# Rudrabha/Wav2Lip

Measured on NVIDIA H100. Metric: 96x96 face-crops/sec (B=128, T=5, mel 80x16), higher is better.
Workload: dtype f16

## Files before the change

wav2lip_b200/csrc/conv_igemm.cuh:

```cuda
#pragma once

#include <cuda.h>
#include <cuda_bf16.h>
#include <cuda_fp16.h>
#include <stdint.h>

#include "wgmma.cuh"

namespace w2l {

constexpr int kTileM = 128;
constexpr int kMaxTaps = 49;
constexpr int kMaxSteps = 3 * kMaxTaps;
constexpr int kSmemExtra = 2048;
constexpr int kSmemMax = 227 * 1024;

enum : int { ACT_NONE = 0, ACT_RELU = 1, ACT_LRELU = 2 };

struct EpiParams {
    int Wout, Hout, N;
    int act;
    int out_f32;
    void* out;
    long long out_sn, out_sy, out_sx;
    const void* res;
    long long res_sn, res_sy, res_sx;
    const float* scale;
    const float* shift;
    const float* head_w;
    const float* head_b;
    int x2;
    int out_lo_off, res_lo_off;
    float* head_out;
    unsigned char* head_out_u8;
    int head_B, head_T;
};

struct alignas(64) ConvParams {
    CUtensorMap tmA;
    CUtensorMap tmB;
    CUtensorMap tmO;
    CUtensorMap tmR;
    int tma_epi;
    unsigned epi_box_bytes;
    int tiles_x, tiles_y, tiles_n, n_tiles;
    int bw, bh, bn;
    int sx, sy;
    int ntaps, kc_per_tap;
    unsigned stage_tx_bytes;
    EpiParams ep;
    int a_lo_off;
    signed char dx[kMaxSteps];
    signed char dy[kMaxSteps];
    unsigned char a_lo[kMaxSteps];
    unsigned char b_slab[kMaxSteps];
};

__device__ __forceinline__ uint32_t smem_u32(const void* p) {
    return static_cast<uint32_t>(__cvta_generic_to_shared(p));
}
__device__ __forceinline__ void mbar_init(uint32_t bar, uint32_t count) {
    asm volatile("mbarrier.init.shared::cta.b64 [%0], %1;" ::"r"(bar), "r"(count) : "memory");
}
__device__ __forceinline__ void mbar_arrive(uint32_t bar) {
    asm volatile("mbarrier.arrive.shared::cta.b64 _, [%0];" ::"r"(bar) : "memory");
}
__device__ __forceinline__ void mbar_arrive_expect_tx(uint32_t bar, uint32_t bytes) {
    asm volatile("mbarrier.arrive.expect_tx.shared::cta.b64 _, [%0], %1;" ::"r"(bar), "r"(bytes) : "memory");
}
__device__ __forceinline__ void mbar_wait(uint32_t bar, uint32_t parity) {
    asm volatile(
        "{\n\t"
        ".reg .pred p;\n\t"
        "W2L_WAIT_%=:\n\t"
        "mbarrier.try_wait.parity.shared::cta.b64 p, [%0], %1;\n\t"
        "@p bra W2L_DONE_%=;\n\t"
        "bra W2L_WAIT_%=;\n\t"
        "W2L_DONE_%=:\n\t"
        "}" ::"r"(bar), "r"(parity)
        : "memory");
}
__device__ __forceinline__ void fence_barrier_init() {
    asm volatile("fence.mbarrier_init.release.cluster;" ::: "memory");
}
__device__ __forceinline__ void tma_prefetch_desc(const void* desc) {
    asm volatile("prefetch.tensormap [%0];" ::"l"(reinterpret_cast<uint64_t>(desc)) : "memory");
}
__device__ __forceinline__ void tma_load_4d(uint32_t dst, const void* desc, uint32_t bar, int c0, int c1, int c2,
                                            int c3) {
    asm volatile(
        "cp.async.bulk.tensor.4d.shared::cluster.global.mbarrier::complete_tx::bytes [%0], [%1, {%3, %4, %5, %6}], [%2];"
        ::"r"(dst), "l"(reinterpret_cast<uint64_t>(desc)), "r"(bar), "r"(c0), "r"(c1), "r"(c2), "r"(c3)
        : "memory");
}
__device__ __forceinline__ void tma_load_3d(uint32_t dst, const void* desc, uint32_t bar, int c0, int c1, int c2) {
    asm volatile(
        "cp.async.bulk.tensor.3d.shared::cluster.global.mbarrier::complete_tx::bytes [%0], [%1, {%3, %4, %5}], [%2];"
        ::"r"(dst), "l"(reinterpret_cast<uint64_t>(desc)), "r"(bar), "r"(c0), "r"(c1), "r"(c2)
        : "memory");
}
__device__ __forceinline__ void pdl_launch_dependents() { asm volatile("griddepcontrol.launch_dependents;" ::: "memory"); }
__device__ __forceinline__ void pdl_wait() { asm volatile("griddepcontrol.wait;" ::: "memory"); }

template <int BK>
__device__ __forceinline__ uint64_t make_kmajor_desc(uint32_t saddr) {
    return wg_desc(saddr, 16, 8 * BK * 2, BK * 2);
}

template <int BN, int BK, bool kBF16>
__device__ __forceinline__ void wg_mma_tile(float (&acc)[2][BN / 2], uint32_t a, uint32_t sbo_a, uint32_t b, bool accumulate) {
#pragma unroll
    for (int k = 0; k < BK / 16; ++k) {
        const uint64_t bd = make_kmajor_desc<BK>(b + 32u * k);
        const uint32_t on = (accumulate || k > 0) ? 1u : 0u;
        wgmma_m64k16<BN, kBF16>(acc[0], wg_desc(a + 32u * k, 16, sbo_a, BK * 2), bd, on, 0);
        wgmma_m64k16<BN, kBF16>(acc[1], wg_desc(a + 8u * sbo_a + 32u * k, 16, sbo_a, BK * 2), bd, on, 0);
    }
}

constexpr int kCmPixels = 256;
template <int BN, int BK, int MT = 1, bool kCM = false>
struct ConvCfg {
    static constexpr int kRowsA = kCM ? kCmPixels : kTileM;
    static constexpr int kATile = kRowsA * BK * 2;
    static constexpr int kABytes = MT * kATile;
    static constexpr int kBBytes = BN * BK * 2;
    static constexpr int kStageBytes = kABytes + kBBytes;
    static constexpr int kEW = BN < 64 ? BN : 64;
    static constexpr int kCW = BN < 32 ? BN : 32;
    static constexpr int kPasses = kCM ? 1 : BN / kEW;
    static constexpr int kBoxBytes = kRowsA * kEW * 2;
    static constexpr int kGrpRaw = (kCM || kPasses * kBoxBytes > xbuf_bytes<kCW>()) ? kPasses * kBoxBytes : xbuf_bytes<kCW>();
    static constexpr int kGrpBytes = (kGrpRaw + 1023) / 1024 * 1024;
    static constexpr int kStagesRaw = (kSmemMax - kSmemExtra - 2 * kGrpBytes) / kStageBytes;
    static constexpr int kStages = kStagesRaw > 8 ? 8 : kStagesRaw;
    static constexpr int kRingBytes = (kStages * kStageBytes + 1023) / 1024 * 1024;
    static constexpr int kSmemBytes = kRingBytes + 2 * kGrpBytes + kSmemExtra;
    static constexpr int kThreads = 384;
    static_assert(BN <= 128, "a warpgroup holds at most 128 fp32 accumulator columns per row");
    static_assert(!kCM || (BN == 128 && BK == 64 && MT == 1), "channel-major form: 128 channels, 128-byte K rows, one tile");
    static_assert(kBoxBytes % 1024 == 0, "staging boxes must keep the 1024-byte swizzle alignment");
    static_assert(kStages >= 2, "need a pipeline");
    static_assert(kSmemBytes <= kSmemMax, "shared-memory carve-up exceeds the per-CTA limit");
};

__device__ int g_f16_overflow = 0;

template <bool kBF16>
__device__ __forceinline__ uint32_t pack2_live(float a, float b, uint32_t live_bits) {
    if constexpr (kBF16) {
        __nv_bfloat162 h = __floats2bfloat162_rn(a, b);
        return *reinterpret_cast<uint32_t*>(&h);
    } else {
        __half2 h = __floats2half2_rn(a, b);
        const uint32_t u = *reinterpret_cast<uint32_t*>(&h);
        if (((u & 0x7FFF7FFFu) + 0x04000400u) & live_bits) g_f16_overflow = 1;
        return u;
    }
}
template <bool kBF16>
__device__ __forceinline__ uint32_t pack2(float a, float b, bool live = true) {
    return pack2_live<kBF16>(a, b, live ? 0x80008000u : 0u);
}
template <bool kBF16>
__device__ __forceinline__ float2 unpack2(uint32_t u) {
    if constexpr (kBF16) {
        return __bfloat1622float2(*reinterpret_cast<__nv_bfloat162*>(&u));
    } else {
        return __half22float2(*reinterpret_cast<__half2*>(&u));
    }
}

template <int BN, bool kBF16, bool kHead>
__device__ __forceinline__ void epilogue_tile(const EpiParams& e, const float (&acc)[2][BN / 2], float* xb, uint32_t bar_id,
                                              bool valid, int n, int y, int x, int nt) {
    constexpr int CH = (BN >= 32) ? 32 : 16;
    const long long o_off = (long long)n * e.out_sn + (long long)y * e.out_sy + (long long)x * e.out_sx;
    const long long r_off = (long long)n * e.res_sn + (long long)y * e.res_sy + (long long)x * e.res_sx;
#pragma unroll
    for (int c0 = 0; c0 < BN; c0 += CH) {
        uint32_t v[CH];
        acc_to_rows<CH>(acc[0], acc[1], c0, xb, bar_id, v);
        if (valid) {
            const int cg = nt * BN + c0;
            float f[CH];
#pragma unroll
            for (int j = 0; j < CH; j += 4) {
                const float4 sc = __ldg(reinterpret_cast<const float4*>(e.scale + cg + j));
                const float4 sh = __ldg(reinterpret_cast<const float4*>(e.shift + cg + j));
                f[j + 0] = fmaf(__uint_as_float(v[j + 0]), sc.x, sh.x);
                f[j + 1] = fmaf(__uint_as_float(v[j + 1]), sc.y, sh.y);
                f[j + 2] = fmaf(__uint_as_float(v[j + 2]), sc.z, sh.z);
                f[j + 3] = fmaf(__uint_as_float(v[j + 3]), sc.w, sh.w);
            }
            if (e.res != nullptr) {
                const uint4* rp = reinterpret_cast<const uint4*>(
                    reinterpret_cast<const uint16_t*>(e.res) + r_off + cg);
#pragma unroll
                for (int j = 0; j < CH / 8; ++j) {
                    const uint4 r = __ldg(rp + j);
                    const float2 a = unpack2<kBF16>(r.x), b = unpack2<kBF16>(r.y);
                    const float2 c = unpack2<kBF16>(r.z), d = unpack2<kBF16>(r.w);
                    f[8 * j + 0] += a.x; f[8 * j + 1] += a.y; f[8 * j + 2] += b.x; f[8 * j + 3] += b.y;
                    f[8 * j + 4] += c.x; f[8 * j + 5] += c.y; f[8 * j + 6] += d.x; f[8 * j + 7] += d.y;
                }
                if (e.x2) {
#pragma unroll
                    for (int j = 0; j < CH / 8; ++j) {
                        const uint4 r = __ldg(rp + (e.res_lo_off >> 3) + j);
                        const float2 a = unpack2<kBF16>(r.x), b = unpack2<kBF16>(r.y);
                        const float2 c = unpack2<kBF16>(r.z), d = unpack2<kBF16>(r.w);
                        f[8 * j + 0] += a.x; f[8 * j + 1] += a.y; f[8 * j + 2] += b.x; f[8 * j + 3] += b.y;
                        f[8 * j + 4] += c.x; f[8 * j + 5] += c.y; f[8 * j + 6] += d.x; f[8 * j + 7] += d.y;
                    }
                }
            }
            if (e.act == ACT_RELU) {
#pragma unroll
                for (int j = 0; j < CH; ++j) f[j] = fmaxf(f[j], 0.0f);
            } else if (e.act == ACT_LRELU) {
#pragma unroll
                for (int j = 0; j < CH; ++j) f[j] = f[j] > 0.0f ? f[j] : 0.01f * f[j];
            }
            if constexpr (kHead) {
                const int hb = n % e.head_B, ht = n / e.head_B;
                const long long plane = (long long)e.Hout * e.Wout;
#pragma unroll
                for (int oc = 0; oc < 3; ++oc) {
                    float s = __ldg(e.head_b + oc);
#pragma unroll
                    for (int j = 0; j < 32; ++j) s = fmaf(f[j], __ldg(e.head_w + oc * 32 + j), s);
                    s = 1.0f / (1.0f + __expf(-s));
                    if (e.head_out_u8 != nullptr)
                        e.head_out_u8[(((long long)n * e.Hout + y) * e.Wout + x) * 3 + oc] = (unsigned char)__fmul_rn(s, 255.0f);
                    else
                        e.head_out[(((long long)hb * 3 + oc) * e.head_T + ht) * plane + (long long)y * e.Wout + x] = s;
                }
            } else if (e.out_f32) {
                float4* op = reinterpret_cast<float4*>(reinterpret_cast<float*>(e.out) + o_off + cg);
#pragma unroll
                for (int j = 0; j < CH / 4; ++j) op[j] = make_float4(f[4 * j], f[4 * j + 1], f[4 * j + 2], f[4 * j + 3]);
            } else {
                uint4* op = reinterpret_cast<uint4*>(reinterpret_cast<uint16_t*>(e.out) + o_off + cg);
#pragma unroll
                for (int j = 0; j < CH / 8; ++j) {
                    uint4 o;
                    o.x = pack2<kBF16>(f[8 * j + 0], f[8 * j + 1]);
                    o.y = pack2<kBF16>(f[8 * j + 2], f[8 * j + 3]);
                    o.z = pack2<kBF16>(f[8 * j + 4], f[8 * j + 5]);
                    o.w = pack2<kBF16>(f[8 * j + 6], f[8 * j + 7]);
                    op[j] = o;
                    if (e.x2) {
                        const float2 h0 = unpack2<kBF16>(o.x), h1 = unpack2<kBF16>(o.y);
                        const float2 h2 = unpack2<kBF16>(o.z), h3 = unpack2<kBF16>(o.w);
                        uint4 l;
                        l.x = pack2<kBF16>(f[8 * j + 0] - h0.x, f[8 * j + 1] - h0.y);
                        l.y = pack2<kBF16>(f[8 * j + 2] - h1.x, f[8 * j + 3] - h1.y);
                        l.z = pack2<kBF16>(f[8 * j + 4] - h2.x, f[8 * j + 5] - h2.y);
                        l.w = pack2<kBF16>(f[8 * j + 6] - h3.x, f[8 * j + 7] - h3.y);
                        op[(e.out_lo_off >> 3) + j] = l;
                    }
                }
            }
        }
    }
}

__device__ __forceinline__ void named_bar_sync(uint32_t id, uint32_t n) { asm volatile("bar.sync %0, %1;" ::"r"(id), "r"(n) : "memory"); }
__device__ __forceinline__ void named_bar_arrive(uint32_t id, uint32_t n) { asm volatile("bar.arrive %0, %1;" ::"r"(id), "r"(n) : "memory"); }

template <bool kBF16, typename AfterRes, typename Live>
__device__ __forceinline__ void chmajor_epilogue(float (&acc)[128], float sc0, float sh0, float sc1, float sh1, int act,
                                                 uint32_t res, int res_pitch, AfterRes&& after_res, Live&& live, uint32_t stg,
                                                 uint32_t bar_id, bool leader, const CUtensorMap* tmO, int c0, int c1, int c2,
                                                 int c3) {
    constexpr uint32_t kRowB = 128;
    const int lane = threadIdx.x & 31, q = (threadIdx.x >> 5) & 3;
    const int lm_row = lane >> 4, lm_px = lane & 7;
    const uint32_t lm_chunk = 16u * (2 * q + ((lane >> 3) & 1));
#pragma unroll
    for (int i = 0; i < 16; ++i) {
#pragma unroll
        for (int h = 0; h < 2; ++h) {
            float* a = acc + 8 * i + 4 * h;
            a[0] = fmaf(a[0], sc0, sh0); a[1] = fmaf(a[1], sc0, sh0);
            a[2] = fmaf(a[2], sc1, sh1); a[3] = fmaf(a[3], sc1, sh1);
        }
        if (res != 0) {
            uint32_t ad = res + static_cast<uint32_t>((2 * i + lm_row) * res_pitch + lm_px) * kRowB + lm_chunk;
            ad ^= ((ad >> 7) & 7u) << 4;
            uint32_t rv[4];
            asm volatile("ldmatrix.sync.aligned.m8n8.x4.trans.shared.b16 {%0,%1,%2,%3}, [%4];"
                         : "=r"(rv[0]), "=r"(rv[1]), "=r"(rv[2]), "=r"(rv[3]) : "r"(ad));
#pragma unroll
            for (int m = 0; m < 4; ++m) {
                const float2 v = unpack2<kBF16>(rv[m]);
                acc[8 * i + 2 * m] += v.x;
                acc[8 * i + 2 * m + 1] += v.y;
            }
        }
    }
    after_res();
    if (act == ACT_RELU) {
#pragma unroll
        for (int j = 0; j < 128; ++j) acc[j] = fmaxf(acc[j], 0.0f);
    } else if (act == ACT_LRELU) {
#pragma unroll
        for (int j = 0; j < 128; ++j) acc[j] = acc[j] > 0.0f ? acc[j] : 0.01f * acc[j];
    }
    if (leader) asm volatile("cp.async.bulk.wait_group.read 0;" ::: "memory");
    named_bar_sync(bar_id, 128);
#pragma unroll
    for (int i = 0; i < 16; ++i) {
        uint32_t ad = stg + static_cast<uint32_t>((2 * i + lm_row) * 8 + lm_px) * kRowB + lm_chunk;
        ad ^= ((ad >> 7) & 7u) << 4;
        const uint32_t l0 = live(2 * i), l1 = live(2 * i + 1);
        const uint32_t o0 = pack2_live<kBF16>(acc[8 * i + 0], acc[8 * i + 1], l0);
        const uint32_t o1 = pack2_live<kBF16>(acc[8 * i + 2], acc[8 * i + 3], l0);
        const uint32_t o2 = pack2_live<kBF16>(acc[8 * i + 4], acc[8 * i + 5], l1);
        const uint32_t o3 = pack2_live<kBF16>(acc[8 * i + 6], acc[8 * i + 7], l1);
        asm volatile("stmatrix.sync.aligned.m8n8.x4.trans.shared.b16 [%0], {%1,%2,%3,%4};"
                     ::"r"(ad), "r"(o0), "r"(o1), "r"(o2), "r"(o3) : "memory");
    }
    asm volatile("fence.proxy.async.shared::cta;" ::: "memory");
    named_bar_sync(bar_id, 128);
    if (leader) {
        asm volatile("cp.async.bulk.tensor.4d.global.shared::cta.bulk_group [%0, {%2, %3, %4, %5}], [%1];"
                     ::"l"(reinterpret_cast<uint64_t>(tmO)), "r"(stg), "r"(c0), "r"(c1), "r"(c2), "r"(c3)
                     : "memory");
        asm volatile("cp.async.bulk.commit_group;" ::: "memory");
    }
}

constexpr int kProducerRegs = 40, kConsumerRegs = 232;
template <int kRegs>
__device__ __forceinline__ void setmaxnreg_dec() { asm volatile("setmaxnreg.dec.sync.aligned.u32 %0;" ::"n"(kRegs)); }
template <int kRegs>
__device__ __forceinline__ void setmaxnreg_inc() { asm volatile("setmaxnreg.inc.sync.aligned.u32 %0;" ::"n"(kRegs)); }

template <int BN, int BK, bool kBF16, bool kHead, int MT = 1, bool kCM = false>
__global__ void __launch_bounds__(ConvCfg<BN, BK, MT, kCM>::kThreads, 1) conv_igemm_kernel(const __grid_constant__ ConvParams p) {
    pdl_launch_dependents();
    using Cfg = ConvCfg<BN, BK, MT, kCM>;
    constexpr int kStages = Cfg::kStages;
    static_assert(!kHead || BN == 32, "fused head expects the 32-channel output block");
    static_assert(MT == 1 || MT == 2, "one or two M tiles per unit");
    static_assert(!kCM || !kHead, "the channel-major form stages its epilogue");

    extern __shared__ uint8_t smem_raw[];
    const uint32_t smem_raw_u32 = smem_u32(smem_raw);
    const uint32_t smem_base = (smem_raw_u32 + 1023u) & ~1023u;
    const uint32_t grp_base = smem_base + Cfg::kRingBytes;
    const uint32_t bar_base = grp_base + 2 * Cfg::kGrpBytes;
    auto full_bar = [&](int s) { return bar_base + 8u * s; };
    auto empty_bar = [&](int s) { return bar_base + 8u * (kStages + s); };
    auto res_bar = [&](int g) { return bar_base + 8u * (2 * kStages + g); };

    const int warp = threadIdx.x >> 5;
    const int lane = threadIdx.x & 31;

    if (warp == 0 && lane == 0) {
        tma_prefetch_desc(&p.tmA);
        tma_prefetch_desc(&p.tmB);
        if (p.tma_epi) {
            tma_prefetch_desc(&p.tmO);
            tma_prefetch_desc(&p.tmR);
        }
    }
    if (warp == 1 && lane == 0) {
        for (int s = 0; s < kStages; ++s) {
            mbar_init(full_bar(s), 1);
            mbar_init(empty_bar(s), kCM ? 8 : 4 * MT);
        }
        for (int g = 0; g < 2; ++g) mbar_init(res_bar(g), 1);
        fence_barrier_init();
    }
    __syncthreads();
    pdl_wait();

    const int m_tiles = p.tiles_x * p.tiles_y * p.tiles_n;
    const int m_units = (m_tiles + MT - 1) / MT;
    const int total_tiles = m_units * p.n_tiles;
    const int k_steps = p.ntaps * p.kc_per_tap;

    if (warp < 4) {
        setmaxnreg_dec<kProducerRegs>();
        if (warp == 0 && lane == 0) {
            int stage = 0;
            uint32_t phase = 0;
            for (int tile = blockIdx.x; tile < total_tiles; tile += gridDim.x) {
                const int nt = tile % p.n_tiles;
                const int mu = tile / p.n_tiles;
                int x_in0[MT], y_in0[MT], n0[MT];
#pragma unroll
                for (int mt = 0; mt < MT; ++mt) {
                    const int m = mu * MT + mt;
                    const int tx = m % p.tiles_x;
                    const int ty = (m / p.tiles_x) % p.tiles_y;
                    const int tn = m / (p.tiles_x * p.tiles_y);
                    x_in0[mt] = tx * p.bw * p.sx;
                    y_in0[mt] = ty * p.bh * p.sy;
                    n0[mt] = tn * p.bn;
                }
                for (int t = 0; t < p.ntaps; ++t) {
                    for (int kc = 0; kc < p.kc_per_tap; ++kc) {
                        mbar_wait(empty_bar(stage), phase ^ 1u);
                        const uint32_t a_dst = smem_base + stage * Cfg::kStageBytes;
                        const uint32_t b_dst = a_dst + Cfg::kABytes;
                        mbar_arrive_expect_tx(full_bar(stage), p.stage_tx_bytes);
#pragma unroll
                        for (int mt = 0; mt < MT; ++mt)
                            tma_load_4d(a_dst + mt * Cfg::kATile, &p.tmA, full_bar(stage), kc * BK + (p.a_lo[t] ? p.a_lo_off : 0),
                                        x_in0[mt] + p.dx[t], y_in0[mt] + p.dy[t], n0[mt]);
                        tma_load_3d(b_dst, &p.tmB, full_bar(stage), kc * BK, nt * BN, p.b_slab[t]);
                        if (++stage == kStages) { stage = 0; phase ^= 1u; }
                    }
                }
            }
        }
    } else if constexpr (kCM) {
        setmaxnreg_inc<kConsumerRegs>();
        const int g = (warp - 4) >> 2;
        const int q = (warp - 4) & 3;
        const uint32_t bar_id = 1 + g;
        const bool leader = (q == 0 && lane == 0);
        const uint32_t stg = grp_base + g * Cfg::kGrpBytes;
        const bool has_res = p.ep.res != nullptr;
        const int rows_valid = p.bw * p.bh * p.bn;
        const int ch = 64 * g + 16 * q + (lane >> 2);
        auto tile_origin = [&](int tile_, int* nt_, int* x0_, int* y0_, int* n0_) {
            *nt_ = tile_ % p.n_tiles;
            const int m_ = tile_ / p.n_tiles;
            *x0_ = (m_ % p.tiles_x) * p.bw;
            *y0_ = ((m_ / p.tiles_x) % p.tiles_y) * p.bh;
            *n0_ = (m_ / (p.tiles_x * p.tiles_y)) * p.bn;
        };
        auto fetch_res = [&](int tile_) {
            int nt_, x0_, y0_, n0_;
            tile_origin(tile_, &nt_, &x0_, &y0_, &n0_);
            mbar_arrive_expect_tx(res_bar(g), p.epi_box_bytes);
            tma_load_4d(stg, &p.tmR, res_bar(g), nt_ * BN + 64 * g, x0_, y0_, n0_);
        };
        if (has_res && leader && static_cast<int>(blockIdx.x) < total_tiles) fetch_res(blockIdx.x);
        float acc[128];
        int stage = 0;
        uint32_t phase = 0, rphase = 0;
        for (int tile = blockIdx.x; tile < total_tiles; tile += gridDim.x) {
            int prev = -1;
            for (int ks = 0; ks < k_steps; ++ks) {
                mbar_wait(full_bar(stage), phase);
                const uint32_t box = smem_base + stage * Cfg::kStageBytes;
                const uint32_t wts = box + Cfg::kABytes + g * (64 * BK * 2);
                wg_fence();
#pragma unroll
                for (int k = 0; k < BK / 16; ++k)
                    wgmma_m64k16<256, kBF16>(acc, make_kmajor_desc<BK>(wts + 32u * k), make_kmajor_desc<BK>(box + 32u * k),
                                             (ks | k) != 0 ? 1u : 0u, 0);
                wg_commit();
                wg_wait<1>();
                if (prev >= 0 && lane == 0) mbar_arrive(empty_bar(prev));
                prev = stage;
                if (++stage == kStages) { stage = 0; phase ^= 1u; }
            }
            wg_wait<0>();
            wg_fence_regs<128>(acc);
            if (lane == 0) mbar_arrive(empty_bar(prev));

            int nt, x0, y0, n0;
            tile_origin(tile, &nt, &x0, &y0, &n0);
            uint64_t live = ~0ull;
            if constexpr (!kBF16) {
                const int xr = p.ep.Wout - x0, yr = p.ep.Hout - y0, nr = p.ep.N - n0;
                if (rows_valid < kCmPixels || xr < p.bw || yr < p.bh || nr < p.bn) {
                    live = 0;
#pragma unroll 1
                    for (int b = 0; b < 64; ++b) {
                        const int px = 8 * (b >> 1) + 2 * (lane & 3) + (b & 1);
                        const int xx = px % p.bw, yy = (px / p.bw) % p.bh, nn = px / (p.bw * p.bh);
                        if (px < rows_valid && xx < xr && yy < yr && nn < nr) live |= 1ull << b;
                    }
                }
            }
            if (has_res) {
                mbar_wait(res_bar(g), rphase);
                rphase ^= 1u;
            }
            const float* const sc = p.ep.scale + nt * BN + ch;
            const float* const sh = p.ep.shift + nt * BN + ch;
            chmajor_epilogue<kBF16>(
                acc, __ldg(sc), __ldg(sh), __ldg(sc + 8), __ldg(sh + 8), p.ep.act, has_res ? stg : 0u, 8, [] {},
                [&](int j) {
                    return (static_cast<uint32_t>(live >> (2 * j)) & 1u) << 15 | (static_cast<uint32_t>(live >> (2 * j + 1)) & 1u) << 31;
                },
                stg, bar_id, leader, &p.tmO, nt * BN + 64 * g, x0, y0, n0);
            if (has_res && leader && tile + static_cast<int>(gridDim.x) < total_tiles) {
                asm volatile("cp.async.bulk.wait_group.read 0;" ::: "memory");
                fetch_res(tile + gridDim.x);
            }
        }
        if (leader) asm volatile("cp.async.bulk.wait_group 0;" ::: "memory");
    } else {
        setmaxnreg_inc<kConsumerRegs>();
        const int g = (warp - 4) >> 2;
        const int q = (warp - 4) & 3;
        const int mt = MT == 2 ? g : 0;
        constexpr int kItStride = MT == 2 ? 1 : 2;
        const int it0 = MT == 2 ? 0 : g;
        const int rows_valid = p.bw * p.bh * p.bn;
        const uint32_t bar_id = 1 + g;
        const uint32_t my_turn = 3 + g, their_turn = 3 + (g ^ 1);
        const uint32_t grp = grp_base + g * Cfg::kGrpBytes;
        float acc[2][BN / 2];
        auto mainloop = [&](int s0, bool hand_off) {
            int stage = s0 % kStages;
            uint32_t phase = static_cast<uint32_t>(s0 / kStages) & 1u;
            int prev = -1;
            for (int ks = 0; ks < k_steps; ++ks) {
                mbar_wait(full_bar(stage), phase);
                const uint32_t a_addr = smem_base + stage * Cfg::kStageBytes + mt * Cfg::kATile;
                wg_fence();
                wg_mma_tile<BN, BK, kBF16>(acc, a_addr, 8 * BK * 2, smem_base + stage * Cfg::kStageBytes + Cfg::kABytes, ks > 0);
                wg_commit();
                wg_wait<1>();
                if (prev >= 0 && lane == 0) mbar_arrive(empty_bar(prev));
                prev = stage;
                if (++stage == kStages) { stage = 0; phase ^= 1u; }
            }
            if (hand_off) named_bar_arrive(their_turn, 256);
            wg_wait<0>();
            wg_fence_regs<BN / 2>(acc[0]);
            wg_fence_regs<BN / 2>(acc[1]);
            if (prev >= 0 && lane == 0) mbar_arrive(empty_bar(prev));
        };
        auto for_each_tile = [&](auto&& epilogue) {
            for (int it = it0;; it += kItStride) {
                const int tile = blockIdx.x + it * static_cast<int>(gridDim.x);
                if (tile >= total_tiles) break;
                if (MT == 1 && it > 0) named_bar_sync(my_turn, 256);
                mainloop(it * k_steps, MT == 1 && tile + static_cast<int>(gridDim.x) < total_tiles);
                epilogue(tile, tile + kItStride * static_cast<int>(gridDim.x) < total_tiles);
            }
        };
        auto tile_origin = [&](int tile_, int* nt_, int* x0_, int* y0_, int* n0_) {
            *nt_ = tile_ % p.n_tiles;
            const int m_ = (tile_ / p.n_tiles) * MT + mt;
            *x0_ = (m_ % p.tiles_x) * p.bw;
            *y0_ = ((m_ / p.tiles_x) % p.tiles_y) * p.bh;
            *n0_ = (m_ / (p.tiles_x * p.tiles_y)) * p.bn;
        };
        if (!kHead && p.tma_epi) {
            constexpr int EW = Cfg::kEW;
            constexpr int kPasses = Cfg::kPasses;
            constexpr uint32_t kRowB = EW * 2;
            constexpr uint32_t kSwz = (kRowB == 128) ? 7u : (kRowB == 64) ? 3u : 1u;
            const bool leader = (q == 0 && lane == 0);
            const bool has_res = p.ep.res != nullptr;
            const EpiParams& e = p.ep;
            auto fetch_res = [&](int tile_) {
                int nt_, x0_, y0_, n0_;
                tile_origin(tile_, &nt_, &x0_, &y0_, &n0_);
                mbar_arrive_expect_tx(res_bar(g), kPasses * p.epi_box_bytes);
#pragma unroll
                for (int ps = 0; ps < kPasses; ++ps)
                    tma_load_4d(grp + ps * Cfg::kBoxBytes, &p.tmR, res_bar(g), nt_ * BN + ps * EW, x0_, y0_, n0_);
            };
            if (has_res && leader) {
                const int first = blockIdx.x + it0 * static_cast<int>(gridDim.x);
                if (first < total_tiles) fetch_res(first);
            }
            uint32_t rphase = 0;
            for_each_tile([&](int tile, bool more) {
                int nt, x0, y0, n0;
                tile_origin(tile, &nt, &x0, &y0, &n0);
                if (has_res) {
                    mbar_wait(res_bar(g), rphase);
                    rphase ^= 1u;
                }
                const float* const scale = e.scale + nt * BN;
                const float* const shift = e.shift + nt * BN;
#pragma unroll
                for (int j = 0; j < BN / 8; ++j) {
                    const int c = 8 * j + 2 * (lane & 3);
                    const float2 sc = __ldg(reinterpret_cast<const float2*>(scale + c));
                    const float2 sh = __ldg(reinterpret_cast<const float2*>(shift + c));
                    const uint32_t box = grp + (8 * j / EW) * Cfg::kBoxBytes;
#pragma unroll
                    for (int h = 0; h < 2; ++h) {
#pragma unroll
                        for (int r8 = 0; r8 < 2; ++r8) {
                            const int row = 64 * h + 16 * q + (lane >> 2) + 8 * r8;
                            float f0 = fmaf(acc[h][4 * j + 2 * r8], sc.x, sh.x);
                            float f1 = fmaf(acc[h][4 * j + 2 * r8 + 1], sc.y, sh.y);
                            uint32_t a = box + row * kRowB + (c % EW) * 2;
                            a ^= ((a >> 7) & kSwz) << 4;
                            if (has_res) {
                                uint32_t r;
                                asm volatile("ld.shared.b32 %0, [%1];" : "=r"(r) : "r"(a));
                                const float2 rv = unpack2<kBF16>(r);
                                f0 += rv.x;
                                f1 += rv.y;
                            }
                            if (e.act == ACT_RELU) {
                                f0 = fmaxf(f0, 0.0f);
                                f1 = fmaxf(f1, 0.0f);
                            } else if (e.act == ACT_LRELU) {
                                f0 = f0 > 0.0f ? f0 : 0.01f * f0;
                                f1 = f1 > 0.0f ? f1 : 0.01f * f1;
                            }
                            const uint32_t o = pack2<kBF16>(f0, f1, row < rows_valid);
                            asm volatile("st.shared.b32 [%0], %1;" ::"r"(a), "r"(o) : "memory");
                        }
                    }
                }
                asm volatile("fence.proxy.async.shared::cta;" ::: "memory");
                named_bar_sync(bar_id, 128);
                if (leader) {
#pragma unroll
                    for (int ps = 0; ps < kPasses; ++ps)
                        asm volatile("cp.async.bulk.tensor.4d.global.shared::cta.bulk_group [%0, {%2, %3, %4, %5}], [%1];"
                                     ::"l"(reinterpret_cast<uint64_t>(&p.tmO)), "r"(grp + ps * Cfg::kBoxBytes), "r"(nt * BN + ps * EW),
                                       "r"(x0), "r"(y0), "r"(n0)
                                     : "memory");
                    asm volatile("cp.async.bulk.commit_group;" ::: "memory");
                    asm volatile("cp.async.bulk.wait_group.read 0;" ::: "memory");
                    if (has_res && more) fetch_res(tile + kItStride * static_cast<int>(gridDim.x));
                }
                if (has_res)
                    __syncwarp();
                else
                    named_bar_sync(bar_id, 128);
            });
            if (leader) asm volatile("cp.async.bulk.wait_group 0;" ::: "memory");
        } else {
            const int row = q * 32 + lane;
            const int px = row % p.bw;
            const int py = (row / p.bw) % p.bh;
            const int pn = row / (p.bw * p.bh);
            float* const xb = reinterpret_cast<float*>(smem_raw + (grp - smem_raw_u32));
            for_each_tile([&](int tile, bool) {
                int nt, x0, y0, n0;
                tile_origin(tile, &nt, &x0, &y0, &n0);
                const int x = x0 + px, y = y0 + py, n = n0 + pn;
                const bool valid = (row < rows_valid) && (x < p.ep.Wout) && (y < p.ep.Hout) && (n < p.ep.N);
                epilogue_tile<BN, kBF16, kHead>(p.ep, acc, xb, bar_id, valid, n, y, x, nt);
            });
        }
    }
}

}
```

wav2lip_b200/csrc/host_launch.cuh:

```cuda
#pragma once

typedef void (*ConvKernelFn)(const ConvParams);
struct ConvKernelEntry { int BN, BK; bool bf16, head; ConvKernelFn fn; int smem; uint64_t attr_set; int mt; int threads; bool cm; };

#define W2L_CONV_ENTRY(BN_, BK_)                                                                                                        \
    {BN_, BK_, false, false, conv_igemm_kernel<BN_, BK_, false, false>, ConvCfg<BN_, BK_>::kSmemBytes, 0, 1, ConvCfg<BN_, BK_>::kThreads, false}, \
    {BN_, BK_, true, false, conv_igemm_kernel<BN_, BK_, true, false>, ConvCfg<BN_, BK_>::kSmemBytes, 0, 1, ConvCfg<BN_, BK_>::kThreads, false}
#define W2L_CONV_ENTRY_MT2(BN_, BK_)                                                                                                    \
    {BN_, BK_, false, false, conv_igemm_kernel<BN_, BK_, false, false, 2>, ConvCfg<BN_, BK_, 2>::kSmemBytes, 0, 2, ConvCfg<BN_, BK_, 2>::kThreads, false}, \
    {BN_, BK_, true, false, conv_igemm_kernel<BN_, BK_, true, false, 2>, ConvCfg<BN_, BK_, 2>::kSmemBytes, 0, 2, ConvCfg<BN_, BK_, 2>::kThreads, false}
#define W2L_CONV_ENTRY_CM(BN_, BK_)                                                                                                     \
    {BN_, BK_, false, false, conv_igemm_kernel<BN_, BK_, false, false, 1, true>, ConvCfg<BN_, BK_, 1, true>::kSmemBytes, 0, 1, ConvCfg<BN_, BK_, 1, true>::kThreads, true}, \
    {BN_, BK_, true, false, conv_igemm_kernel<BN_, BK_, true, false, 1, true>, ConvCfg<BN_, BK_, 1, true>::kSmemBytes, 0, 1, ConvCfg<BN_, BK_, 1, true>::kThreads, true}

static ConvKernelEntry g_conv_kernels[] = {
    W2L_CONV_ENTRY(16, 16), W2L_CONV_ENTRY(16, 32), W2L_CONV_ENTRY(16, 64),
    W2L_CONV_ENTRY(32, 16), W2L_CONV_ENTRY(32, 32), W2L_CONV_ENTRY(32, 64),
    W2L_CONV_ENTRY(64, 16), W2L_CONV_ENTRY(64, 32), W2L_CONV_ENTRY(64, 64),
    W2L_CONV_ENTRY(128, 16), W2L_CONV_ENTRY(128, 32), W2L_CONV_ENTRY(128, 64),
    W2L_CONV_ENTRY_MT2(64, 64), W2L_CONV_ENTRY_MT2(64, 32),
    W2L_CONV_ENTRY_CM(128, 64),
    {32, 16, false, true, conv_igemm_kernel<32, 16, false, true>, ConvCfg<32, 16>::kSmemBytes, 0, 1, ConvCfg<32, 16>::kThreads, false},
    {32, 16, true, true, conv_igemm_kernel<32, 16, true, true>, ConvCfg<32, 16>::kSmemBytes, 0, 1, ConvCfg<32, 16>::kThreads, false},
};

static ConvKernelEntry* find_conv_kernel(int BN, int BK, bool bf16, bool head, int mt = 1, bool cm = false) {
    for (auto& e : g_conv_kernels)
        if (e.BN == BN && e.BK == BK && e.bf16 == bf16 && e.head == head && e.mt == mt && e.cm == cm) return &e;
    return nullptr;
}

typedef void (*PatchKernelFn)(const PatchParams);
struct PatchKernelEntry { int BN, BK; bool bf16, head; PatchKernelFn fn; uint64_t attr_set; };
#define W2L_PATCH_ENTRY(BN_, BK_)                                                    \
    {BN_, BK_, false, false, conv_patch_kernel<BN_, BK_, false, false>, 0},    \
    {BN_, BK_, true, false, conv_patch_kernel<BN_, BK_, true, false>, 0}
static PatchKernelEntry g_patch_kernels[] = {
    W2L_PATCH_ENTRY(16, 16), W2L_PATCH_ENTRY(16, 32), W2L_PATCH_ENTRY(16, 64),
    W2L_PATCH_ENTRY(32, 16), W2L_PATCH_ENTRY(32, 32), W2L_PATCH_ENTRY(32, 64),
    W2L_PATCH_ENTRY(64, 16), W2L_PATCH_ENTRY(64, 32), W2L_PATCH_ENTRY(64, 64),
    {32, 16, false, true, conv_patch_kernel<32, 16, false, true>, 0},
    {32, 16, true, true, conv_patch_kernel<32, 16, true, true>, 0},
};
static PatchKernelEntry* find_patch_kernel(int BN, int BK, bool bf16, bool head) {
    for (auto& e : g_patch_kernels)
        if (e.BN == BN && e.BK == BK && e.bf16 == bf16 && e.head == head) return &e;
    return nullptr;
}

typedef void (*CtKernelFn)(const ConvTParams);
struct CtKernelEntry { int BK; bool bf16; CtKernelFn fn; uint64_t attr_set; };
static CtKernelEntry g_ct_kernels[] = {
    {32, false, convt_fused_kernel<32, false>, 0}, {32, true, convt_fused_kernel<32, true>, 0},
};
constexpr int kCtSmemMax = 227 * 1024;

static int ensure_smem_attr(uint64_t* mask, int device, const void* fn, int bytes) {
    const uint64_t bit = 1ull << (device & 63);
    if (*mask & bit) return W2L_OK;
    CK(cudaFuncSetAttribute(fn, cudaFuncAttributeMaxDynamicSharedMemorySize, bytes));
    *mask |= bit;
    return W2L_OK;
}

template <typename P>
static cudaError_t launch_k(void (*fn)(const P), int grid, int block, size_t smem, cudaStream_t st, const P& p, bool pdl) {
    cudaLaunchConfig_t cfg;
    memset(&cfg, 0, sizeof(cfg));
    cfg.gridDim = dim3((unsigned)grid, 1, 1);
    cfg.blockDim = dim3((unsigned)block, 1, 1);
    cfg.dynamicSmemBytes = smem;
    cfg.stream = st;
    cudaLaunchAttribute at[1];
    at[0].id = cudaLaunchAttributeProgrammaticStreamSerialization;
    at[0].val.programmaticStreamSerializationAllowed = 1;
    cfg.attrs = at;
    cfg.numAttrs = pdl ? 1 : 0;
    return cudaLaunchKernelEx(&cfg, fn, p);
}

static void op_kernel_info(const w2l_ctx* ctx, const Op& op, w2l_kernel_info* k) {
    memset(k, 0, sizeof(*k));
    snprintf(k->name, sizeof(k->name), "%s", op.name.c_str());
    k->family = op.ctf ? W2L_KFAM_CONVT_FUSED : op.patch ? W2L_KFAM_PATCH : W2L_KFAM_IGEMM;
    k->bn = op.BN; k->bk = op.BK; k->mt = op.MT; k->head = op.head ? 1 : 0;
    k->bf16 = ctx->bf16 ? 1 : 0; k->x2 = ctx->x2 ? 1 : 0;
    k->tma_epi = (!op.ctf && !op.patch && op.cp.tma_epi) ? 1 : 0;
    k->fold = op.fold ? 1 : 0;
    k->m_tiles = op.m_tiles; k->n_tiles = op.n_tiles; k->grid = op.grid;
}

static int launch_conv(w2l_ctx* ctx, const Op& op, cudaStream_t st, bool pdl = true) {
    pdl = pdl && ctx->use_pdl;
    if (op.ctf) {
        CtKernelEntry* e = nullptr;
        for (auto& k : g_ct_kernels) if (k.BK == op.BK && k.bf16 == ctx->bf16) e = &k;
        if (!e) return fail(W2L_EINVAL, "no fused convT kernel for BK=%d", op.BK);
        CKR(ensure_smem_attr(&e->attr_set, ctx->device, (const void*)e->fn, kCtSmemMax));
        CK(launch_k(e->fn, op.grid, kCtThreads, op.dyn_smem, st, op.tp, pdl));
        ctx->launches++;
        return W2L_OK;
    }
    if (op.patch) {
        PatchKernelEntry* e = find_patch_kernel(op.BN, op.BK, ctx->bf16, op.head);
        if (!e) return fail(W2L_EINVAL, "no patch kernel for BN=%d BK=%d head=%d", op.BN, op.BK, (int)op.head);
        CKR(ensure_smem_attr(&e->attr_set, ctx->device, (const void*)e->fn, kSmemMax));
        CK(launch_k(e->fn, op.grid, kPatchThreads, op.dyn_smem, st, op.pp, pdl));
        ctx->launches++;
        return W2L_OK;
    }
    ConvKernelEntry* e = find_conv_kernel(op.BN, op.BK, ctx->bf16, op.head, op.MT, op.cm);
    if (!e) return fail(W2L_EINVAL, "no conv kernel for BN=%d BK=%d head=%d MT=%d cm=%d", op.BN, op.BK, (int)op.head, op.MT, (int)op.cm);
    CKR(ensure_smem_attr(&e->attr_set, ctx->device, (const void*)e->fn, e->smem));
    CK(launch_k(e->fn, op.grid, e->threads, (size_t)e->smem, st, op.cp, pdl));
    ctx->launches++;
    return W2L_OK;
}
```

wav2lip_b200/csrc/host_ops.cuh:

```cuda
#pragma once

static int pick_bk(int cin_pad) { return (cin_pad % 64 == 0) ? 64 : (cin_pad % 32 == 0) ? 32 : 16; }
static int round_up(int a, int b) { return (a + b - 1) / b * b; }
constexpr int kCmMinSteps = 18;
constexpr int kCmMinCtaSteps = 48;
constexpr double kCmFillMargin = 0.06;

static void pick_box(int W, int H, int N, int sx, int sy, int* bw, int* bh, int* bn, int pixels = kTileM) {
    double best = 1e30;
    int b_w = 1, b_h = 1, b_n = 1;
    for (int w = 1; w <= std::min(W, pixels); ++w) {
        if (w * sx > 256) break;
        for (int h = 1; h <= std::min(H, pixels / w); ++h) {
            if (h * sy > 256) break;
            int n = std::min(pixels / (w * h), std::max(N, 1));
            if (n < 1) continue;
            if (n > 256) n = 256;
            const double tiles = (double)((W + w - 1) / w) * ((H + h - 1) / h) * ((N + n - 1) / n);
            const double cost = tiles - 1e-6 * w - 1e-9 * h;
            if (cost < best) { best = cost; b_w = w; b_h = h; b_n = n; }
        }
    }
    *bw = b_w; *bh = b_h; *bn = b_n;
}

struct ConvArgs {
    std::string name;
    Act in, out;
    const PackedW* w = nullptr;
    int sx = 1, sy = 1;
    int Hl = 0, Wl = 0;
    int osy = 1, osx = 1;
    int phy = 0, phx = 0;
    const Act* res = nullptr;
    const float* scale = nullptr;
    const float* shift = nullptr;
    int ch_off = 0;
    int act = ACT_RELU;
    int cout = 0;
    double macs_per_pixel = 0;
    bool head = false;
    const float* head_w = nullptr;
    const float* head_b = nullptr;
    int head_B = 1, head_T = 1;
};

static void fill_epi(EpiParams* e, const ConvArgs& a) {
    memset(e, 0, sizeof(*e));
    e->Wout = a.Wl; e->Hout = a.Hl; e->N = a.in.N;
    e->act = a.act;
    e->out_f32 = a.out.f32 ? 1 : 0;
    const long long oCs = a.out.Cs;
    const long long Wfull = a.out.W;
    if (!a.head) {
        const long long base_off = ((long long)a.phy * Wfull + a.phx) * oCs + a.out.c_off;
        e->out = a.out.f32 ? (void*)((float*)a.out.base + base_off) : (void*)(a.out.base + base_off);
        e->out_sn = (long long)a.out.H * Wfull * oCs;
        e->out_sy = (long long)a.osy * Wfull * oCs;
        e->out_sx = (long long)a.osx * oCs;
    }
    if (a.res) {
        const long long rCs = a.res->Cs, rW = a.res->W;
        e->res = a.res->ptr() + ((long long)a.phy * rW + a.phx) * rCs;
        e->res_sn = (long long)a.res->H * rW * rCs;
        e->res_sy = (long long)a.osy * rW * rCs;
        e->res_sx = (long long)a.osx * rCs;
    }
    e->scale = a.scale + a.ch_off;
    e->shift = a.shift + a.ch_off;
    e->head_w = a.head_w; e->head_b = a.head_b; e->head_out = nullptr; e->head_B = a.head_B; e->head_T = a.head_T;
    e->x2 = (a.out.lo_off > 0 || (a.res && a.res->lo_off > 0)) ? 1 : 0;
    e->out_lo_off = a.out.lo_off;
    e->res_lo_off = a.res ? a.res->lo_off : 0;
}

static int encode_act_map(w2l_ctx* ctx, CUtensorMap* tm, const Act& in, int BK, int bx, int by, int bn, int sx, int sy,
                          const char* name) {
    EncodeTiledFn enc = get_encode_fn();
    const CUtensorMapDataType dt = ctx->bf16 ? CU_TENSOR_MAP_DATA_TYPE_BFLOAT16 : CU_TENSOR_MAP_DATA_TYPE_FLOAT16;
    const CUtensorMapSwizzle sw = BK == 64 ? CU_TENSOR_MAP_SWIZZLE_128B : BK == 32 ? CU_TENSOR_MAP_SWIZZLE_64B : CU_TENSOR_MAP_SWIZZLE_32B;
    cuuint64_t dims[4] = {(cuuint64_t)(in.lo_off + in.C), (cuuint64_t)(in.nwin ? in.nwin : in.W), (cuuint64_t)in.H, (cuuint64_t)in.N};
    cuuint64_t strides[3] = {(cuuint64_t)in.Cs * in.wstride * 2, (cuuint64_t)in.pitch() * in.Cs * 2, (cuuint64_t)in.H * in.pitch() * in.Cs * 2};
    cuuint32_t box[4] = {(cuuint32_t)BK, (cuuint32_t)bx, (cuuint32_t)by, (cuuint32_t)bn};
    cuuint32_t es[4] = {1, (cuuint32_t)sx, (cuuint32_t)sy, 1};
    CUresult r = enc(tm, dt, 4, in.ptr(), dims, strides, box, es, CU_TENSOR_MAP_INTERLEAVE_NONE, sw,
                     CU_TENSOR_MAP_L2_PROMOTION_L2_128B, CU_TENSOR_MAP_FLOAT_OOB_FILL_NONE);
    if (r != CUDA_SUCCESS)
        return fail(W2L_ECUDA, "%s: cuTensorMapEncodeTiled(A) failed with %d (dims %d,%d,%d,%d box %d,%d,%d,%d)", name, (int)r,
                    in.C, in.W, in.H, in.N, BK, bx, by, bn);
    return W2L_OK;
}

static int encode_w_map(w2l_ctx* ctx, CUtensorMap* tm, const PackedW& w, int BK, int BN, const char* name) {
    EncodeTiledFn enc = get_encode_fn();
    const CUtensorMapDataType dt = ctx->bf16 ? CU_TENSOR_MAP_DATA_TYPE_BFLOAT16 : CU_TENSOR_MAP_DATA_TYPE_FLOAT16;
    const CUtensorMapSwizzle sw = BK == 64 ? CU_TENSOR_MAP_SWIZZLE_128B : BK == 32 ? CU_TENSOR_MAP_SWIZZLE_64B : CU_TENSOR_MAP_SWIZZLE_32B;
    cuuint64_t dims[3] = {(cuuint64_t)w.cin_pad, (cuuint64_t)w.cout_pad, (cuuint64_t)(w.nslabs ? w.nslabs : w.ntaps)};
    cuuint64_t strides[2] = {(cuuint64_t)w.cin_pad * 2, (cuuint64_t)w.cin_pad * w.cout_pad * 2};
    cuuint32_t box[3] = {(cuuint32_t)BK, (cuuint32_t)BN, 1};
    cuuint32_t es[3] = {1, 1, 1};
    CUresult r = enc(tm, dt, 3, w.w, dims, strides, box, es, CU_TENSOR_MAP_INTERLEAVE_NONE, sw,
                     CU_TENSOR_MAP_L2_PROMOTION_L2_256B, CU_TENSOR_MAP_FLOAT_OOB_FILL_NONE);
    if (r != CUDA_SUCCESS) return fail(W2L_ECUDA, "%s: cuTensorMapEncodeTiled(B) failed with %d", name, (int)r);
    return W2L_OK;
}

struct PatchGeom { int ox, oy, PW, PH, BK, TH, patch_bytes, patch_stride, wbytes, stg_bytes, res_tap; };

constexpr int kPatchSmemBudget = kSmemMax - kSmemExtra;

static bool patch_eligible(const w2l_ctx* ctx, const ConvArgs& a, PatchGeom* g) {
    if (!ctx->use_patch) return false;
    const PackedW& w = *a.w;
    if (a.sx != 1 || a.sy != 1 || w.ntaps > kPatchMaxTaps) return false;
    if (a.cout != 16 && a.cout != 32 && a.cout != 64) return false;
    if (w.cout_pad != a.cout) return false;
    if (a.head && a.cout != 32) return false;
    if (a.Wl < kPatchTileW || a.Hl < kPatchTileW) return false;
    if (a.out.f32) return false;
    g->BK = pick_bk(w.cin_pad);
    g->TH = patch_chmajor(a.cout, g->BK, a.head) ? kChTileH : kPatchTileH;
    const double tiles = (double)((a.Wl + kPatchTileW - 1) / kPatchTileW) * ((a.Hl + g->TH - 1) / g->TH);
    if ((double)a.Wl * a.Hl / (tiles * kPatchTileW * g->TH) < 0.6) return false;
    int mnx = 127, mxx = -127, mny = 127, mxy = -127;
    for (int t = 0; t < w.ntaps; ++t) {
        mnx = std::min(mnx, (int)w.dx[t]); mxx = std::max(mxx, (int)w.dx[t]);
        mny = std::min(mny, (int)w.dy[t]); mxy = std::max(mxy, (int)w.dy[t]);
    }
    g->ox = mnx; g->oy = mny;
    g->PW = kPatchTileW + (mxx - mnx); g->PH = g->TH + (mxy - mny);
    g->patch_bytes = g->PW * g->PH * g->BK * 2;
    g->patch_stride = (g->patch_bytes + 1023) / 1024 * 1024;
    g->wbytes = w.ntaps * w.cin_pad * a.cout * 2;
    g->stg_bytes = 2 * ((kPatchTileW * g->TH * a.cout * 2 + 1023) / 1024 * 1024);
    if (g->PW > 256 || g->PH > 256) return false;
    if (g->wbytes + g->stg_bytes + 2 * (w.cin_pad / g->BK) * g->patch_stride > kPatchSmemBudget) return false;
    g->res_tap = -1;
    if (a.res) {
        if (a.res->base != a.in.base || a.res->c_off != a.in.c_off || a.res->Cs != a.in.Cs) return false;
        if (w.cin_pad != a.cout || w.cin_pad != g->BK) return false;
        for (int t = 0; t < w.ntaps; ++t)
            if (w.dx[t] == 0 && w.dy[t] == 0) g->res_tap = t;
        if (g->res_tap < 0) return false;
    }
    return true;
}

static int make_patch_op(w2l_ctx* ctx, Plan* pl, const ConvArgs& a, const PatchGeom& g) {
    Op op;
    op.type = OP_CONV;
    op.name = a.name + (a.w->fold ? " [fold+patch]" : " [patch]");
    op.patch = true;
    op.head = a.head;
    const PackedW& w = *a.w;
    const int BK = g.BK, BN = a.cout;
    op.BN = BN; op.BK = BK;
    PatchParams& h = op.pp;
    memset(&h, 0, sizeof(h));
    CKR(encode_act_map(ctx, &h.tmA, a.in, BK, g.PW, g.PH, 1, 1, 1, a.name.c_str()));
    CKR(encode_w_map(ctx, &h.tmB, w, BK, BN, a.name.c_str()));
    h.tiles_x = (a.Wl + kPatchTileW - 1) / kPatchTileW;
    h.tiles_y = (a.Hl + g.TH - 1) / g.TH;
    h.kc = w.cin_pad / BK;
    h.PW = g.PW; h.PH = g.PH; h.ox = g.ox; h.oy = g.oy;
    h.ntaps = w.ntaps;
    h.patch_bytes = g.patch_bytes; h.patch_stride = g.patch_stride;
    for (int t = 0; t < w.ntaps; ++t) h.tap_row[t] = (w.dy[t] - g.oy) * g.PW + (w.dx[t] - g.ox);
    h.stages = std::min(kPatchMaxStages, (kPatchSmemBudget - g.wbytes - g.stg_bytes) / (h.kc * g.patch_stride)) & ~1;
    op.dyn_smem = g.wbytes + h.stages * h.kc * g.patch_stride + g.stg_bytes + kSmemExtra;
    if (op.dyn_smem > kSmemMax || h.stages < 2) return fail(W2L_EINVAL, "%s: patch kernel smem plan %d B / %d stages", a.name.c_str(), op.dyn_smem, h.stages);
    fill_epi(&h.ep, a);
    h.res_row = g.res_tap >= 0 ? h.tap_row[g.res_tap] : -1;
    if (!a.head) {
        EncodeTiledFn enc = get_encode_fn();
        const CUtensorMapDataType dt = ctx->bf16 ? CU_TENSOR_MAP_DATA_TYPE_BFLOAT16 : CU_TENSOR_MAP_DATA_TYPE_FLOAT16;
        const CUtensorMapSwizzle sw = BN == 64 ? CU_TENSOR_MAP_SWIZZLE_128B : BN == 32 ? CU_TENSOR_MAP_SWIZZLE_64B : CU_TENSOR_MAP_SWIZZLE_32B;
        cuuint64_t dims[4] = {(cuuint64_t)BN, (cuuint64_t)a.Wl, (cuuint64_t)a.Hl, (cuuint64_t)a.in.N};
        cuuint64_t strides[3] = {(cuuint64_t)h.ep.out_sx * 2, (cuuint64_t)h.ep.out_sy * 2, (cuuint64_t)h.ep.out_sn * 2};
        cuuint32_t box[4] = {(cuuint32_t)BN, (cuuint32_t)kPatchTileW, (cuuint32_t)g.TH, 1};
        cuuint32_t es[4] = {1, 1, 1, 1};
        if (a.out.f32) return fail(W2L_EINVAL, "%s: patch kernel stores 16-bit outputs only", a.name.c_str());
        CUresult r = enc(&h.tmO, dt, 4, h.ep.out, dims, strides, box, es, CU_TENSOR_MAP_INTERLEAVE_NONE, sw,
                         CU_TENSOR_MAP_L2_PROMOTION_L2_128B, CU_TENSOR_MAP_FLOAT_OOB_FILL_NONE);
        if (r != CUDA_SUCCESS) return fail(W2L_ECUDA, "%s: cuTensorMapEncodeTiled(out) failed with %d", a.name.c_str(), (int)r);
    } else {
        h.tmO = h.tmA;
    }
    CK(cudaDeviceSynchronize());
    CK(cudaMemcpy(h.cscale, a.scale + a.ch_off, (size_t)BN * 4, cudaMemcpyDeviceToHost));
    CK(cudaMemcpy(h.cshift, a.shift + a.ch_off, (size_t)BN * 4, cudaMemcpyDeviceToHost));
    if (a.head) {
        CK(cudaMemcpy(h.chead_w, a.head_w, 96 * 4, cudaMemcpyDeviceToHost));
        CK(cudaMemcpy(h.chead_b, a.head_b, 3 * 4, cudaMemcpyDeviceToHost));
    }
    const long long total = (long long)h.tiles_x * h.tiles_y * a.in.N;
    op.grid = (int)std::min<long long>(total, ctx->num_sms);
    op.fold = w.fold; op.m_tiles = (int)total; op.n_tiles = 1;
    op.flops = 2.0 * a.macs_per_pixel * (double)a.Wl * a.Hl * a.in.N;
    pl->ops.push_back(op);
    return W2L_OK;
}

static int make_conv_op(w2l_ctx* ctx, Plan* pl, const ConvArgs& a) {
    if (!get_encode_fn()) return fail(W2L_ENODEV, "cuTensorMapEncodeTiled is not available (no CUDA driver?)");
    const PackedW& w = *a.w;
    if (a.in.C != w.cin_pad) return fail(W2L_EINVAL, "%s: input view has %d channels, weights packed for %d", a.name.c_str(), a.in.C, w.cin_pad);
    if (a.cout % 16 != 0) return fail(W2L_EINVAL, "%s: cout %d not a multiple of 16", a.name.c_str(), a.cout);
    PatchGeom geom;
    if (patch_eligible(ctx, a, &geom)) return make_patch_op(ctx, pl, a, geom);
    Op op;
    op.type = OP_CONV;
    op.name = a.name + (w.fold ? " [fold]" : "");
    const int BK = pick_bk(w.cin_pad);
    int bw, bh, bn;
    pick_box(a.Wl, a.Hl, a.in.N, a.sx, a.sy, &bw, &bh, &bn);
    int tiles_x = (a.Wl + bw - 1) / bw, tiles_y = (a.Hl + bh - 1) / bh, tiles_n = (a.in.N + bn - 1) / bn;
    int m_tiles = tiles_x * tiles_y * tiles_n;
    int BN = 16;
    for (int cand : {128, 64, 32, 16})
        if (a.cout % cand == 0) { BN = cand; break; }
    if (a.head) BN = 32;
    else
        while (BN > 32 && m_tiles * (a.cout / BN) < ctx->num_sms && a.cout % (BN / 2) == 0) BN /= 2;
    const int k_steps = w.ntaps * (w.cin_pad / BK);
    if (ctx->use_tma_epi && !ctx->x2 && !a.head && !a.out.f32 && a.cout % 128 == 0 && w.cout_pad % 128 == 0 && BK == 64 &&
        a.osx == 1 && a.osy == 1 && k_steps >= kCmMinSteps) {
        int cw, ch, cn;
        pick_box(a.Wl, a.Hl, a.in.N, a.sx, a.sy, &cw, &ch, &cn, kCmPixels);
        const long long cm_tiles = (long long)((a.Wl + cw - 1) / cw) * ((a.Hl + ch - 1) / ch) * ((a.in.N + cn - 1) / cn);
        const int S = ctx->num_sms, nt = a.cout / 128;
        auto fill = [&](long long tiles, int pixels) {
            const long long rounds = (tiles * nt + S - 1) / S;
            return (double)a.Wl * a.Hl * a.in.N / ((double)rounds * S * pixels / nt);
        };
        if ((cm_tiles * nt + S - 1) / S * k_steps >= kCmMinCtaSteps &&
            fill(cm_tiles, kCmPixels) >= (1.0 - kCmFillMargin) * fill(m_tiles, kTileM)) {
            op.cm = true;
            op.name += " [cm]";
            BN = 128;
            bw = cw; bh = ch; bn = cn;
            tiles_x = (a.Wl + bw - 1) / bw; tiles_y = (a.Hl + bh - 1) / bh; tiles_n = (a.in.N + bn - 1) / bn;
            m_tiles = tiles_x * tiles_y * tiles_n;
        }
    }
    if (w.cout_pad % BN != 0) return fail(W2L_EINVAL, "%s: cout_pad %d vs BN %d", a.name.c_str(), w.cout_pad, BN);
    op.BN = BN; op.BK = BK; op.head = a.head;
    const int n_tiles_ = a.cout / BN;
    if (ctx->use_mt2 && !a.head && !op.cm && find_conv_kernel(BN, BK, ctx->bf16, false, 2) &&
        (long long)((m_tiles + 1) / 2) * n_tiles_ >= 2LL * ctx->num_sms)
        op.MT = 2;
    if (op.MT == 2) op.name += " [2M]";

    ConvParams& p = op.cp;
    memset(&p, 0, sizeof(p));
    CKR(encode_act_map(ctx, &p.tmA, a.in, BK, bw * a.sx, bh * a.sy, bn, a.sx, a.sy, a.name.c_str()));
    CKR(encode_w_map(ctx, &p.tmB, w, BK, BN, a.name.c_str()));
    p.tiles_x = tiles_x; p.tiles_y = tiles_y; p.tiles_n = tiles_n; p.n_tiles = a.cout / BN;
    p.bw = bw; p.bh = bh; p.bn = bn;
    p.sx = a.sx; p.sy = a.sy;
    p.ntaps = w.ntaps; p.kc_per_tap = w.cin_pad / BK;
    p.stage_tx_bytes = (unsigned)(op.MT * bw * bh * bn * BK * 2 + BN * BK * 2);
    fill_epi(&p.ep, a);
    p.tma_epi = 0;
    if (ctx->use_tma_epi && !ctx->x2 && !a.head && !a.out.f32) {
        EncodeTiledFn enc = get_encode_fn();
        const int EW = BN < 64 ? BN : 64;
        const CUtensorMapDataType dt = ctx->bf16 ? CU_TENSOR_MAP_DATA_TYPE_BFLOAT16 : CU_TENSOR_MAP_DATA_TYPE_FLOAT16;
        const CUtensorMapSwizzle esw = EW == 64 ? CU_TENSOR_MAP_SWIZZLE_128B : EW == 32 ? CU_TENSOR_MAP_SWIZZLE_64B : CU_TENSOR_MAP_SWIZZLE_32B;
        cuuint64_t dims[4] = {(cuuint64_t)std::min(a.cout, a.out.C), (cuuint64_t)a.Wl, (cuuint64_t)a.Hl, (cuuint64_t)a.in.N};
        cuuint32_t box[4] = {(cuuint32_t)EW, (cuuint32_t)bw, (cuuint32_t)bh, (cuuint32_t)bn};
        cuuint32_t es[4] = {1, 1, 1, 1};
        cuuint64_t os[3] = {(cuuint64_t)p.ep.out_sx * 2, (cuuint64_t)p.ep.out_sy * 2, (cuuint64_t)p.ep.out_sn * 2};
        CUresult r = enc(&p.tmO, dt, 4, p.ep.out, dims, os, box, es, CU_TENSOR_MAP_INTERLEAVE_NONE, esw,
                         CU_TENSOR_MAP_L2_PROMOTION_L2_128B, CU_TENSOR_MAP_FLOAT_OOB_FILL_NONE);
        if (r != CUDA_SUCCESS) return fail(W2L_ECUDA, "%s: cuTensorMapEncodeTiled(out) failed with %d", a.name.c_str(), (int)r);
        if (a.res) {
            cuuint64_t rs[3] = {(cuuint64_t)p.ep.res_sx * 2, (cuuint64_t)p.ep.res_sy * 2, (cuuint64_t)p.ep.res_sn * 2};
            r = enc(&p.tmR, dt, 4, const_cast<void*>(p.ep.res), dims, rs, box, es, CU_TENSOR_MAP_INTERLEAVE_NONE, esw,
                    CU_TENSOR_MAP_L2_PROMOTION_L2_128B, CU_TENSOR_MAP_FLOAT_OOB_FILL_NONE);
            if (r != CUDA_SUCCESS) return fail(W2L_ECUDA, "%s: cuTensorMapEncodeTiled(res) failed with %d", a.name.c_str(), (int)r);
        } else {
            p.tmR = p.tmO;
        }
        p.tma_epi = 1;
        p.epi_box_bytes = (unsigned)(bw * bh * bn * EW * 2);
    }
    if (w.ntaps > kMaxTaps) return fail(W2L_EINVAL, "%s: too many taps", a.name.c_str());
    if (a.cout > a.out.C && !p.tma_epi && !a.head) return fail(W2L_ESTATE, "%s: %d computed channels for a %d-channel destination need the TMA-store epilogue", a.name.c_str(), a.cout, a.out.C);
    if (ctx->x2) {
        if (a.in.lo_off <= 0 || w.nslabs != 2 * w.ntaps) return fail(W2L_ESTATE, "%s: split-operand mode needs hi/lo planes", a.name.c_str());
        int k = 0;
        for (int t = 0; t < w.ntaps; ++t)
            for (int v = 0; v < 3; ++v, ++k) {
                p.dx[k] = w.dx[t]; p.dy[k] = w.dy[t];
                p.a_lo[k] = (v == 1) ? 1 : 0;
                p.b_slab[k] = (unsigned char)((v == 2) ? w.ntaps + t : t);
            }
        p.ntaps = 3 * w.ntaps;
        p.a_lo_off = a.in.lo_off;
    } else {
        for (int t = 0; t < w.ntaps; ++t) { p.dx[t] = w.dx[t]; p.dy[t] = w.dy[t]; p.a_lo[t] = 0; p.b_slab[t] = (unsigned char)t; }
    }
    const int total = ((m_tiles + op.MT - 1) / op.MT) * p.n_tiles;
    op.grid = std::min(total, ctx->num_sms);
    op.fold = w.fold; op.m_tiles = m_tiles; op.n_tiles = p.n_tiles;
    op.flops = 2.0 * a.macs_per_pixel * (double)a.Wl * a.Hl * a.in.N;
    pl->ops.push_back(op);
    return W2L_OK;
}

static int make_convt_fused_op(w2l_ctx* ctx, Plan* pl, const Layer& L, const LayerW& lw, const Act& in, const Act& out, int act = ACT_RELU) {
    EncodeTiledFn enc = get_encode_fn();
    if (!enc) return fail(W2L_ENODEV, "cuTensorMapEncodeTiled is not available");
    const PackedW& w = lw.ph.back();
    Op op;
    op.type = OP_CONV;
    op.name = L.name + " [fused 4-phase]";
    op.ctf = true;
    const int BK = 32;
    if (w.cin_pad % BK != 0) return fail(W2L_EINVAL, "%s: fused convT needs cin %% 32 == 0", L.name.c_str());
    op.BK = BK; op.BN = kCtBN;
    ConvTParams& t = op.tp;
    memset(&t, 0, sizeof(t));
    CKR(encode_act_map(ctx, &t.tmA, in, BK, kCtPW, kCtPH, 1, 1, 1, L.name.c_str()));
    {
        const CUtensorMapDataType dt = ctx->bf16 ? CU_TENSOR_MAP_DATA_TYPE_BFLOAT16 : CU_TENSOR_MAP_DATA_TYPE_FLOAT16;
        const CUtensorMapSwizzle sw = CU_TENSOR_MAP_SWIZZLE_64B;
        cuuint64_t dims[3] = {(cuuint64_t)w.cin_pad, (cuuint64_t)w.cout_pad, 9};
        cuuint64_t strides[2] = {(cuuint64_t)w.cin_pad * 2, (cuuint64_t)w.cin_pad * w.cout_pad * 2};
        cuuint32_t box[3] = {(cuuint32_t)BK, (cuuint32_t)kCtBN, 9};
        cuuint32_t es[3] = {1, 1, 1};
        CUresult r = enc(&t.tmB, dt, 3, w.w, dims, strides, box, es, CU_TENSOR_MAP_INTERLEAVE_NONE, sw,
                         CU_TENSOR_MAP_L2_PROMOTION_L2_256B, CU_TENSOR_MAP_FLOAT_OOB_FILL_NONE);
        if (r != CUDA_SUCCESS) return fail(W2L_ECUDA, "%s: cuTensorMapEncodeTiled(B9) failed with %d", L.name.c_str(), (int)r);
        for (int py = 0; py < 2; ++py)
            for (int px = 0; px < 2; ++px) {
                uint16_t* base = out.base + ((long long)py * out.W + px) * out.Cs + out.c_off;
                cuuint64_t od[4] = {(cuuint64_t)kCtBN, (cuuint64_t)in.W, (cuuint64_t)in.H, (cuuint64_t)in.N};
                cuuint64_t os[3] = {(cuuint64_t)2 * out.Cs * 2, (cuuint64_t)2 * out.W * out.Cs * 2, (cuuint64_t)out.H * out.W * out.Cs * 2};
                cuuint32_t ob[4] = {(cuuint32_t)kCtBN, 8, 16, 1};
                cuuint32_t oe[4] = {1, 1, 1, 1};
                CUresult r2 = enc(&t.tmO[py * 2 + px], dt, 4, base, od, os, ob, oe, CU_TENSOR_MAP_INTERLEAVE_NONE,
                                  CU_TENSOR_MAP_SWIZZLE_128B, CU_TENSOR_MAP_L2_PROMOTION_L2_128B, CU_TENSOR_MAP_FLOAT_OOB_FILL_NONE);
                if (r2 != CUDA_SUCCESS) return fail(W2L_ECUDA, "%s: cuTensorMapEncodeTiled(out phase) failed with %d", L.name.c_str(), (int)r2);
            }
    }
    t.tiles_x = (in.W + 7) / 8; t.tiles_y = (in.H + 15) / 16; t.N = in.N;
    t.kc = w.cin_pad / BK;
    t.patch_bytes = kCtPW * kCtPH * BK * 2;
    t.patch_stride = (t.patch_bytes + 1023) / 1024 * 1024;
    const int stage_bytes = t.patch_stride + 9 * kCtBN * BK * 2;
    const int fixed = 2 * kTileM * kCtBN * 2 + kSmemExtra;
    t.stages = std::min(kCtMaxStages, (kCtSmemMax - fixed) / stage_bytes);
    if (t.stages < 2) return fail(W2L_EINVAL, "%s: fused convT does not fit shared memory", L.name.c_str());
    op.dyn_smem = t.stages * stage_bytes + fixed;
    t.act = act;
    CK(cudaDeviceSynchronize());
    CK(cudaMemcpy(t.cscale, lw.scale, kCtBN * 4, cudaMemcpyDeviceToHost));
    CK(cudaMemcpy(t.cshift, lw.shift, kCtBN * 4, cudaMemcpyDeviceToHost));
    const long long units = (long long)t.tiles_x * t.tiles_y * in.N;
    op.grid = (int)std::min<long long>(units, ctx->num_sms);
    op.m_tiles = (int)units; op.n_tiles = 1;
    op.flops = 2.0 * (double)L.cin * L.cout * 9 * (double)in.W * in.H * in.N;
    pl->ops.push_back(op);
    return W2L_OK;
}

static int emit_block(w2l_ctx* ctx, Plan* pl, const NetW& nw, int li, const Layer& L, const Act& in, const Act& out,
                      const Act* res, bool head = false, int head_B = 1, int head_T = 1, int act_override = -1) {
    const LayerW& lw = nw.layers[li];
    ConvArgs a;
    a.in = in; a.out = out; a.res = res;
    a.scale = lw.scale; a.shift = lw.shift;
    a.act = (L.kind == W2L_BLOCK_CONV_LRELU) ? ACT_LRELU : (L.kind == W2L_BLOCK_CONV_PLAIN ? ACT_NONE : ACT_RELU);
    if (act_override >= 0) a.act = act_override;
    a.cout = L.cout;
    a.head = head; a.head_w = nw.head_w; a.head_b = nw.head_b; a.head_B = head_B; a.head_T = head_T;
    if (L.kind != W2L_BLOCK_CONVT_BN_RELU) {
        a.name = L.name;
        a.w = &lw.ph[0];
        a.sx = lw.ph[0].fold ? 1 : L.sw; a.sy = L.sh;
        a.Hl = out.H; a.Wl = out.W;
        a.macs_per_pixel = (double)L.cin * L.cout * L.kh * L.kw;
        return make_conv_op(ctx, pl, a);
    }
    if (lw.gemm_convT) {
        Act o = out;
        o.H = 1; o.W = 1; o.Cs = out.Cs * out.H * out.W; o.C = L.cout * L.kh * L.kw;
        if (out.c_off != 0 || out.C != out.Cs) return fail(W2L_EINVAL, "%s: gemm convT needs a dense output", L.name.c_str());
        a.name = L.name;
        a.out = o;
        a.w = &lw.ph[0];
        a.Hl = 1; a.Wl = 1;
        a.cout = L.cout * L.kh * L.kw;
        a.macs_per_pixel = (double)L.cin * L.cout * L.kh * L.kw;
        return make_conv_op(ctx, pl, a);
    }
    if (lw.has_all_taps && ctx->use_ctfused && lw.ph.back().cin_pad % 32 == 0 && in.W >= 8 && in.H >= 8 && !res &&
        out.H == 2 * in.H && out.W == 2 * in.W &&
        (double)in.W * in.H / ((double)((in.W + 7) / 8) * ((in.H + 15) / 16) * kTileM) >= 0.6 && !out.f32)
        return make_convt_fused_op(ctx, pl, L, lw, in, out, a.act);
    const size_t nph = lw.ph.size() - (lw.has_all_taps ? 1 : 0);
    for (size_t i = 0; i < nph; ++i) {
        const PackedW& w = lw.ph[i];
        ConvArgs b = a;
        b.name = L.name + ".ph" + std::to_string(w.py) + std::to_string(w.px);
        b.w = &w;
        b.osy = L.sh; b.osx = L.sw; b.phy = w.py; b.phx = w.px;
        b.Hl = (out.H - w.py + L.sh - 1) / L.sh;
        b.Wl = (out.W - w.px + L.sw - 1) / L.sw;
        b.macs_per_pixel = (double)L.cin * L.cout * w.ntaps;
        CKR(make_conv_op(ctx, pl, b));
    }
    return W2L_OK;
}

static void conv_out_dims(const Layer& L, int H, int W, int* Ho, int* Wo) {
    if (L.kind == W2L_BLOCK_CONVT_BN_RELU) {
        *Ho = (H - 1) * L.sh - 2 * L.ph + L.kh + L.out_pad;
        *Wo = (W - 1) * L.sw - 2 * L.pw + L.kw + L.out_pad;
    } else {
        *Ho = (H + 2 * L.ph - L.kh) / L.sh + 1;
        *Wo = (W + 2 * L.pw - L.kw) / L.sw + 1;
    }
}
```

wav2lip_b200/csrc/host_types.h:

```cpp
#pragma once

static thread_local std::string g_err;

static int fail(int code, const char* fmt, ...) {
    char buf[1024];
    va_list ap;
    va_start(ap, fmt);
    vsnprintf(buf, sizeof(buf), fmt, ap);
    va_end(ap);
    g_err = buf;
    return code;
}

#define CK(call)                                                                                         \
    do {                                                                                                 \
        cudaError_t e_ = (call);                                                                         \
        if (e_ != cudaSuccess)                                                                           \
            return fail(W2L_ECUDA, "%s failed: %s (%s:%d)", #call, cudaGetErrorString(e_), __FILE__, __LINE__); \
    } while (0)
#define CKR(expr)               \
    do {                        \
        int r_ = (expr);        \
        if (r_ != W2L_OK) return r_; \
    } while (0)

static const GeneratorSpec& gen_spec() { static GeneratorSpec s = build_generator_spec(); return s; }
static const SyncnetSpec& sync_spec() { static SyncnetSpec s = build_syncnet_spec(); return s; }
static const DiscSpec& disc_spec() { static DiscSpec s = build_disc_spec(); return s; }
static const S3fdSpec& s3fd_spec() { static S3fdSpec s = build_s3fd_spec(); return s; }
static const std::vector<Layer>* net_layers(int net) {
    switch (net) {
        case W2L_NET_GENERATOR: return &gen_spec().layers;
        case W2L_NET_SYNCNET: return &sync_spec().layers;
        case W2L_NET_DISC: return &disc_spec().layers;
        case W2L_NET_S3FD: return &s3fd_spec().layers;
    }
    return nullptr;
}

typedef CUresult (*EncodeTiledFn)(CUtensorMap*, CUtensorMapDataType, cuuint32_t, void*, const cuuint64_t*,
                                  const cuuint64_t*, const cuuint32_t*, const cuuint32_t*, CUtensorMapInterleave,
                                  CUtensorMapSwizzle, CUtensorMapL2promotion, CUtensorMapFloatOOBfill);
static EncodeTiledFn get_encode_fn() {
    static EncodeTiledFn fn = nullptr;
    if (!fn) {
        void* p = nullptr;
        cudaDriverEntryPointQueryResult q;
        if (cudaGetDriverEntryPoint("cuTensorMapEncodeTiled", &p, cudaEnableDefault, &q) == cudaSuccess &&
            q == cudaDriverEntryPointSuccess)
            fn = reinterpret_cast<EncodeTiledFn>(p);
    }
    return fn;
}

struct DeviceGuard {
    int prev = -1;
    explicit DeviceGuard(int dev) { cudaGetDevice(&prev); if (prev != dev) cudaSetDevice(dev); else prev = -1; }
    ~DeviceGuard() { if (prev >= 0) cudaSetDevice(prev); }
};

static int dev_alloc(void** p, size_t bytes) {
    cudaError_t e = cudaMalloc(p, bytes);
    if (e == cudaSuccess) return W2L_OK;
    cudaGetLastError();
    *p = nullptr;
    return fail(W2L_ENOMEM, "cudaMalloc(%zu) failed: %s", bytes, cudaGetErrorString(e));
}

struct w2l_ctx;

template <class T = void>
struct DevMem {
    T* p = nullptr;
    size_t cap = 0;
    size_t* counter = nullptr;
    DevMem() = default;
    DevMem(DevMem&& o) noexcept : p(o.p), cap(o.cap), counter(o.counter) { o.p = nullptr; o.cap = 0; }
    DevMem& operator=(DevMem&& o) noexcept { std::swap(p, o.p); std::swap(cap, o.cap); std::swap(counter, o.counter); return *this; }
    ~DevMem() { if (p) { cudaFree(p); *counter -= cap; } }
    operator T*() const { return p; }
    int grow(w2l_ctx* ctx, size_t bytes);
};

struct Stream {
    cudaStream_t h = nullptr;
    Stream() = default;
    Stream(const Stream&) = delete;
    Stream& operator=(const Stream&) = delete;
    ~Stream() { if (h) cudaStreamDestroy(h); }
    int create() { CK(cudaStreamCreateWithFlags(&h, cudaStreamNonBlocking)); return W2L_OK; }
    operator cudaStream_t() const { return h; }
};

struct Event {
    cudaEvent_t h = nullptr;
    Event() = default;
    Event(const Event&) = delete;
    Event& operator=(const Event&) = delete;
    ~Event() { if (h) cudaEventDestroy(h); }
    int create(unsigned flags = cudaEventDisableTiming) { CK(cudaEventCreateWithFlags(&h, flags)); return W2L_OK; }
    operator cudaEvent_t() const { return h; }
};

struct Act {
    uint16_t* base = nullptr;
    int N = 0, H = 0, W = 0;
    int Cs = 0;
    int c_off = 0;
    int C = 0;
    bool f32 = false;
    int Wp = 0;
    int x_off = 0;
    int lo_off = 0;
    int wstride = 1;
    int nwin = 0;
    int pitch() const { return Wp ? Wp : W; }
    uint16_t* ptr() const { return base + c_off; }
    Act slice(int off, int c) const { Act a = *this; a.c_off = c_off + off; a.C = c; return a; }
};

struct PackedW {
    uint16_t* w = nullptr;
    int ntaps = 0, cout_pad = 0, cin_pad = 0;
    int nslabs = 0;
    std::vector<signed char> dx, dy;
    int py = 0, px = 0;
    bool fold = false;
    int Cp = 0, kfold = 0, win = 0;
};

struct LayerW {
    std::vector<PackedW> ph;
    float* scale = nullptr;
    float* shift = nullptr;
    std::vector<DevMem<>> mem;
    int n_scale = 0;
    bool gemm_convT = false;
    bool has_all_taps = false;
    bool loaded = false;
};

struct NetW {
    std::vector<LayerW> layers;
    DevMem<float> head_w;
    DevMem<float> head_b;
    bool loaded = false;
};

enum OpType { OP_CONV = 0, OP_INGEST = 1, OP_L2NORM = 2, OP_DISC_HEAD = 3, OP_MAXPOOL = 4, OP_CHAN_L2NORM = 5, OP_S3FD_EXPORT = 6 };

struct Op {
    int type = OP_CONV;
    std::string name;
    ConvParams cp;
    int BN = 0, BK = 0, MT = 1;
    bool cm = false;
    bool head = false;
    int grid = 0;
    double flops = 0;
    bool patch = false;
    PatchParams pp;
    int dyn_smem = 0;
    bool ctf = false;
    ConvTParams tp;
    bool fold = false;
    int m_tiles = 0, n_tiles = 0;
    IngestParams ip;
    int ingest_src = 0;
    const void* aux_in = nullptr;
    int aux_rows = 0, aux_dim = 0;
    int aux_out = 0;
    int aux_pitch = 0, aux_lo = 0;
    const uint16_t* sp_in = nullptr; uint16_t* sp_out = nullptr; const float* sp_f32 = nullptr; const float* sp_w = nullptr;
    int sp_N = 0, sp_H = 0, sp_W = 0, sp_C = 0, sp_Cout = 0, sp_maxout = 0;
    int lane = 0;
    bool join_side = false;
};

struct S3fdDetWork {
    S3fdDetParams p;
    bool last = false;
};

struct Plan {
    explicit Plan(w2l_ctx* c) : ctx(c) {}
    w2l_ctx* ctx;
    int net = 0, B = 0, T = 0, N = 0;
    int H = 0, W = 0;
    std::vector<Op> ops;
    std::vector<DevMem<>> allocs;
    std::map<int, Act> layer_out;
    long long last_used = 0;
    int pins = 0;
    bool x2 = false;
    bool has_side = false;
    std::unique_ptr<S3fdDetWork> det;
};

struct FoldJob { const float* bias; int cout, reps, n_pad; float* scale; float* shift; };
struct RepackLog { std::vector<PackParams> pack; std::vector<PackFoldParams> pack_fold; std::vector<FoldJob> fold; };
struct TrainState;

struct w2l_ctx {
    size_t device_bytes = 0;
    int device = 0;
    bool bf16 = false;
    bool x2 = false;
    int num_sms = 132;
    bool keep_all = false;
    bool use_patch = true;
    bool use_mt2 = true;
    bool use_aux_stream = true;
    bool use_wg_stream = true;
    bool use_tma_epi = true;
    bool use_fold_s2 = true;
    bool use_ctfused = true;
    bool use_fold = true;
    bool use_pdl = true;
    bool use_stream_graph = true;
    NetW nets[4];
    DevMem<float> s3fd_l2w[3];
    std::map<std::string, std::unique_ptr<Plan>> plans;
    Plan* last_plan[4] = {nullptr, nullptr, nullptr, nullptr};
    uint64_t plan_epoch[4] = {0, 0, 0, 0};
    std::vector<w2l_kernel_info> last_block_kernels;
    int64_t launches = 0;
    long long plan_clock = 0;
    Stream stream;
    Stream s_h2d, s_d2h;
    Stream s_side;
    Event ev_fork, ev_join;
    bool use_side = true;
    Event ev_in[2], ev_done[2], ev_out[2];
    DevMem<> stage[6];
    DevMem<int> boxes_dev;
    DevMem<int> samples_dev;
    DevMem<uint8_t> crops_dev, preds_dev;
    DevMem<float> scratch;
    long long host_seq = 0;
    int host_inflight = 0;
    DevMem<double2> mel_tw;
    DevMem<float> mel_bvals;
    DevMem<int> mel_boff;
    DevMem<int> mel_bstart;
    DevMem<int> mel_blen;
    std::unique_ptr<TrainState> train;
};

template <class T>
int DevMem<T>::grow(w2l_ctx* ctx, size_t bytes) {
    if (p && cap >= bytes) return W2L_OK;
    if (p) {
        CK(cudaDeviceSynchronize());
        *this = DevMem();
    }
    const size_t n = bytes ? bytes : 16;
    void* q;
    CKR(dev_alloc(&q, n));
    p = (T*)q; cap = n; counter = &ctx->device_bytes;
    *counter += n;
    return W2L_OK;
}

template <class T>
static int alloc_in(w2l_ctx* ctx, std::vector<DevMem<>>* owner, T** p, size_t bytes) {
    owner->emplace_back();
    CKR(owner->back().grow(ctx, bytes));
    *p = (T*)owner->back().p;
    return W2L_OK;
}

template <class T>
static int plan_alloc(Plan* pl, T** p, size_t bytes) { return alloc_in(pl->ctx, &pl->allocs, p, bytes); }

static int plan_act(Plan* pl, Act* a, int N, int H, int W, int C, bool f32 = false) {
    const bool planes = pl->x2 && !f32;
    const size_t bytes = (size_t)N * H * W * C * (f32 ? 4 : 2) * (planes ? 2 : 1);
    CKR(plan_alloc(pl, &a->base, bytes));
    a->N = N; a->H = H; a->W = W; a->Cs = planes ? 2 * C : C; a->c_off = 0; a->C = C; a->f32 = f32;
    a->lo_off = planes ? C : 0;
    return W2L_OK;
}

static int plan_input_act(Plan* pl, Act* a, int N, int H, int W, int cin, const LayerW& lw, const Layer& L) {
    const PackedW& w = lw.ph[0];
    if (!w.fold) return plan_act(pl, a, N, H, W, ((cin + 15) / 16) * 16);
    const int Wout = (W + 2 * L.pw - L.kw) / L.sw + 1;
    const int Wp = (std::max(W + L.pw, (Wout - 1) * L.sw + w.win) + 1) / 2 * 2;
    const size_t bytes = ((size_t)N * H * Wp * w.Cp + w.kfold) * 2;
    CKR(plan_alloc(pl, &a->base, bytes));
    CK(cudaMemset(a->base, 0, bytes));
    a->N = N; a->H = H; a->W = W; a->Cs = w.Cp; a->c_off = 0; a->C = w.kfold; a->f32 = false;
    a->Wp = Wp; a->x_off = L.pw;
    a->wstride = L.sw; a->nwin = Wout;
    return W2L_OK;
}
```

wav2lip_b200/csrc/wgmma.cuh:

```cuda
#pragma once

#include <stdint.h>

namespace w2l {

__device__ __forceinline__ uint64_t wg_desc(uint32_t saddr, uint32_t lbo, uint32_t sbo, uint32_t row_bytes) {
    const uint64_t layout = row_bytes == 128 ? 1 : row_bytes == 64 ? 2 : 3;
    uint64_t d = static_cast<uint64_t>((saddr & 0x3FFFFu) >> 4);
    d |= static_cast<uint64_t>((lbo >> 4) & 0x3FFFu) << 16;
    d |= static_cast<uint64_t>((sbo >> 4) & 0x3FFFu) << 32;
    d |= layout << 62;
    return d;
}

__device__ __forceinline__ void wg_fence() { asm volatile("wgmma.fence.sync.aligned;" ::: "memory"); }
__device__ __forceinline__ void wg_commit() { asm volatile("wgmma.commit_group.sync.aligned;" ::: "memory"); }
template <int kPending>
__device__ __forceinline__ void wg_wait() { asm volatile("wgmma.wait_group.sync.aligned %0;" ::"n"(kPending) : "memory"); }
template <int kRegs>
__device__ __forceinline__ void wg_fence_regs(float* d) {
#pragma unroll
    for (int i = 0; i < kRegs; ++i) asm volatile("" : "+f"(d[i])::"memory");
}

template <int N, bool kBF16>
__device__ __forceinline__ void wgmma_m64k16(float* d, uint64_t a, uint64_t b, uint32_t acc, int tnsp);

template <>
__device__ __forceinline__ void wgmma_m64k16<16, false>(float* d, uint64_t a, uint64_t b, uint32_t acc, int tnsp) {
    if (tnsp)
        asm volatile("{\n.reg .pred p;\nsetp.ne.b32 p, %10, 0;\n"
                     "wgmma.mma_async.sync.aligned.m64n16k16.f32.f16.f16 {%0,%1,%2,%3,%4,%5,%6,%7}, %8, %9, p, 1, 1, 1, 1;\n}"
                     : "+f"(d[0]), "+f"(d[1]), "+f"(d[2]), "+f"(d[3]), "+f"(d[4]), "+f"(d[5]), "+f"(d[6]), "+f"(d[7])
                     : "l"(a), "l"(b), "r"(acc));
    else
        asm volatile("{\n.reg .pred p;\nsetp.ne.b32 p, %10, 0;\n"
                     "wgmma.mma_async.sync.aligned.m64n16k16.f32.f16.f16 {%0,%1,%2,%3,%4,%5,%6,%7}, %8, %9, p, 1, 1, 0, 0;\n}"
                     : "+f"(d[0]), "+f"(d[1]), "+f"(d[2]), "+f"(d[3]), "+f"(d[4]), "+f"(d[5]), "+f"(d[6]), "+f"(d[7])
                     : "l"(a), "l"(b), "r"(acc));
}

template <>
__device__ __forceinline__ void wgmma_m64k16<16, true>(float* d, uint64_t a, uint64_t b, uint32_t acc, int tnsp) {
    if (tnsp)
        asm volatile("{\n.reg .pred p;\nsetp.ne.b32 p, %10, 0;\n"
                     "wgmma.mma_async.sync.aligned.m64n16k16.f32.bf16.bf16 {%0,%1,%2,%3,%4,%5,%6,%7}, %8, %9, p, 1, 1, 1, 1;\n}"
                     : "+f"(d[0]), "+f"(d[1]), "+f"(d[2]), "+f"(d[3]), "+f"(d[4]), "+f"(d[5]), "+f"(d[6]), "+f"(d[7])
                     : "l"(a), "l"(b), "r"(acc));
    else
        asm volatile("{\n.reg .pred p;\nsetp.ne.b32 p, %10, 0;\n"
                     "wgmma.mma_async.sync.aligned.m64n16k16.f32.bf16.bf16 {%0,%1,%2,%3,%4,%5,%6,%7}, %8, %9, p, 1, 1, 0, 0;\n}"
                     : "+f"(d[0]), "+f"(d[1]), "+f"(d[2]), "+f"(d[3]), "+f"(d[4]), "+f"(d[5]), "+f"(d[6]), "+f"(d[7])
                     : "l"(a), "l"(b), "r"(acc));
}

template <>
__device__ __forceinline__ void wgmma_m64k16<32, false>(float* d, uint64_t a, uint64_t b, uint32_t acc, int tnsp) {
    if (tnsp)
        asm volatile("{\n.reg .pred p;\nsetp.ne.b32 p, %18, 0;\n"
                     "wgmma.mma_async.sync.aligned.m64n32k16.f32.f16.f16 {%0,%1,%2,%3,%4,%5,%6,%7,%8,%9,%10,%11,%12,%13,%14,%15}, %16, %17, p, 1, 1, 1, 1;\n}"
                     : "+f"(d[0]), "+f"(d[1]), "+f"(d[2]), "+f"(d[3]), "+f"(d[4]), "+f"(d[5]), "+f"(d[6]), "+f"(d[7]), "+f"(d[8]), "+f"(d[9]), "+f"(d[10]), "+f"(d[11]), "+f"(d[12]), "+f"(d[13]), "+f"(d[14]), "+f"(d[15])
                     : "l"(a), "l"(b), "r"(acc));
    else
        asm volatile("{\n.reg .pred p;\nsetp.ne.b32 p, %18, 0;\n"
                     "wgmma.mma_async.sync.aligned.m64n32k16.f32.f16.f16 {%0,%1,%2,%3,%4,%5,%6,%7,%8,%9,%10,%11,%12,%13,%14,%15}, %16, %17, p, 1, 1, 0, 0;\n}"
                     : "+f"(d[0]), "+f"(d[1]), "+f"(d[2]), "+f"(d[3]), "+f"(d[4]), "+f"(d[5]), "+f"(d[6]), "+f"(d[7]), "+f"(d[8]), "+f"(d[9]), "+f"(d[10]), "+f"(d[11]), "+f"(d[12]), "+f"(d[13]), "+f"(d[14]), "+f"(d[15])
                     : "l"(a), "l"(b), "r"(acc));
}

template <>
__device__ __forceinline__ void wgmma_m64k16<32, true>(float* d, uint64_t a, uint64_t b, uint32_t acc, int tnsp) {
    if (tnsp)
        asm volatile("{\n.reg .pred p;\nsetp.ne.b32 p, %18, 0;\n"
                     "wgmma.mma_async.sync.aligned.m64n32k16.f32.bf16.bf16 {%0,%1,%2,%3,%4,%5,%6,%7,%8,%9,%10,%11,%12,%13,%14,%15}, %16, %17, p, 1, 1, 1, 1;\n}"
                     : "+f"(d[0]), "+f"(d[1]), "+f"(d[2]), "+f"(d[3]), "+f"(d[4]), "+f"(d[5]), "+f"(d[6]), "+f"(d[7]), "+f"(d[8]), "+f"(d[9]), "+f"(d[10]), "+f"(d[11]), "+f"(d[12]), "+f"(d[13]), "+f"(d[14]), "+f"(d[15])
                     : "l"(a), "l"(b), "r"(acc));
    else
        asm volatile("{\n.reg .pred p;\nsetp.ne.b32 p, %18, 0;\n"
                     "wgmma.mma_async.sync.aligned.m64n32k16.f32.bf16.bf16 {%0,%1,%2,%3,%4,%5,%6,%7,%8,%9,%10,%11,%12,%13,%14,%15}, %16, %17, p, 1, 1, 0, 0;\n}"
                     : "+f"(d[0]), "+f"(d[1]), "+f"(d[2]), "+f"(d[3]), "+f"(d[4]), "+f"(d[5]), "+f"(d[6]), "+f"(d[7]), "+f"(d[8]), "+f"(d[9]), "+f"(d[10]), "+f"(d[11]), "+f"(d[12]), "+f"(d[13]), "+f"(d[14]), "+f"(d[15])
                     : "l"(a), "l"(b), "r"(acc));
}

template <>
__device__ __forceinline__ void wgmma_m64k16<64, false>(float* d, uint64_t a, uint64_t b, uint32_t acc, int tnsp) {
    if (tnsp)
        asm volatile("{\n.reg .pred p;\nsetp.ne.b32 p, %34, 0;\n"
                     "wgmma.mma_async.sync.aligned.m64n64k16.f32.f16.f16 {%0,%1,%2,%3,%4,%5,%6,%7,%8,%9,%10,%11,%12,%13,%14,%15,%16,%17,%18,%19,%20,%21,%22,%23,%24,%25,%26,%27,%28,%29,%30,%31}, %32, %33, p, 1, 1, 1, 1;\n}"
                     : "+f"(d[0]), "+f"(d[1]), "+f"(d[2]), "+f"(d[3]), "+f"(d[4]), "+f"(d[5]), "+f"(d[6]), "+f"(d[7]), "+f"(d[8]), "+f"(d[9]), "+f"(d[10]), "+f"(d[11]), "+f"(d[12]), "+f"(d[13]), "+f"(d[14]), "+f"(d[15]), "+f"(d[16]), "+f"(d[17]), "+f"(d[18]), "+f"(d[19]), "+f"(d[20]), "+f"(d[21]), "+f"(d[22]), "+f"(d[23]), "+f"(d[24]), "+f"(d[25]), "+f"(d[26]), "+f"(d[27]), "+f"(d[28]), "+f"(d[29]), "+f"(d[30]), "+f"(d[31])
                     : "l"(a), "l"(b), "r"(acc));
    else
        asm volatile("{\n.reg .pred p;\nsetp.ne.b32 p, %34, 0;\n"
                     "wgmma.mma_async.sync.aligned.m64n64k16.f32.f16.f16 {%0,%1,%2,%3,%4,%5,%6,%7,%8,%9,%10,%11,%12,%13,%14,%15,%16,%17,%18,%19,%20,%21,%22,%23,%24,%25,%26,%27,%28,%29,%30,%31}, %32, %33, p, 1, 1, 0, 0;\n}"
                     : "+f"(d[0]), "+f"(d[1]), "+f"(d[2]), "+f"(d[3]), "+f"(d[4]), "+f"(d[5]), "+f"(d[6]), "+f"(d[7]), "+f"(d[8]), "+f"(d[9]), "+f"(d[10]), "+f"(d[11]), "+f"(d[12]), "+f"(d[13]), "+f"(d[14]), "+f"(d[15]), "+f"(d[16]), "+f"(d[17]), "+f"(d[18]), "+f"(d[19]), "+f"(d[20]), "+f"(d[21]), "+f"(d[22]), "+f"(d[23]), "+f"(d[24]), "+f"(d[25]), "+f"(d[26]), "+f"(d[27]), "+f"(d[28]), "+f"(d[29]), "+f"(d[30]), "+f"(d[31])
                     : "l"(a), "l"(b), "r"(acc));
}

template <>
__device__ __forceinline__ void wgmma_m64k16<64, true>(float* d, uint64_t a, uint64_t b, uint32_t acc, int tnsp) {
    if (tnsp)
        asm volatile("{\n.reg .pred p;\nsetp.ne.b32 p, %34, 0;\n"
                     "wgmma.mma_async.sync.aligned.m64n64k16.f32.bf16.bf16 {%0,%1,%2,%3,%4,%5,%6,%7,%8,%9,%10,%11,%12,%13,%14,%15,%16,%17,%18,%19,%20,%21,%22,%23,%24,%25,%26,%27,%28,%29,%30,%31}, %32, %33, p, 1, 1, 1, 1;\n}"
                     : "+f"(d[0]), "+f"(d[1]), "+f"(d[2]), "+f"(d[3]), "+f"(d[4]), "+f"(d[5]), "+f"(d[6]), "+f"(d[7]), "+f"(d[8]), "+f"(d[9]), "+f"(d[10]), "+f"(d[11]), "+f"(d[12]), "+f"(d[13]), "+f"(d[14]), "+f"(d[15]), "+f"(d[16]), "+f"(d[17]), "+f"(d[18]), "+f"(d[19]), "+f"(d[20]), "+f"(d[21]), "+f"(d[22]), "+f"(d[23]), "+f"(d[24]), "+f"(d[25]), "+f"(d[26]), "+f"(d[27]), "+f"(d[28]), "+f"(d[29]), "+f"(d[30]), "+f"(d[31])
                     : "l"(a), "l"(b), "r"(acc));
    else
        asm volatile("{\n.reg .pred p;\nsetp.ne.b32 p, %34, 0;\n"
                     "wgmma.mma_async.sync.aligned.m64n64k16.f32.bf16.bf16 {%0,%1,%2,%3,%4,%5,%6,%7,%8,%9,%10,%11,%12,%13,%14,%15,%16,%17,%18,%19,%20,%21,%22,%23,%24,%25,%26,%27,%28,%29,%30,%31}, %32, %33, p, 1, 1, 0, 0;\n}"
                     : "+f"(d[0]), "+f"(d[1]), "+f"(d[2]), "+f"(d[3]), "+f"(d[4]), "+f"(d[5]), "+f"(d[6]), "+f"(d[7]), "+f"(d[8]), "+f"(d[9]), "+f"(d[10]), "+f"(d[11]), "+f"(d[12]), "+f"(d[13]), "+f"(d[14]), "+f"(d[15]), "+f"(d[16]), "+f"(d[17]), "+f"(d[18]), "+f"(d[19]), "+f"(d[20]), "+f"(d[21]), "+f"(d[22]), "+f"(d[23]), "+f"(d[24]), "+f"(d[25]), "+f"(d[26]), "+f"(d[27]), "+f"(d[28]), "+f"(d[29]), "+f"(d[30]), "+f"(d[31])
                     : "l"(a), "l"(b), "r"(acc));
}

template <>
__device__ __forceinline__ void wgmma_m64k16<128, false>(float* d, uint64_t a, uint64_t b, uint32_t acc, int tnsp) {
    if (tnsp)
        asm volatile("{\n.reg .pred p;\nsetp.ne.b32 p, %66, 0;\n"
                     "wgmma.mma_async.sync.aligned.m64n128k16.f32.f16.f16 {%0,%1,%2,%3,%4,%5,%6,%7,%8,%9,%10,%11,%12,%13,%14,%15,%16,%17,%18,%19,%20,%21,%22,%23,%24,%25,%26,%27,%28,%29,%30,%31,%32,%33,%34,%35,%36,%37,%38,%39,%40,%41,%42,%43,%44,%45,%46,%47,%48,%49,%50,%51,%52,%53,%54,%55,%56,%57,%58,%59,%60,%61,%62,%63}, %64, %65, p, 1, 1, 1, 1;\n}"
                     : "+f"(d[0]), "+f"(d[1]), "+f"(d[2]), "+f"(d[3]), "+f"(d[4]), "+f"(d[5]), "+f"(d[6]), "+f"(d[7]), "+f"(d[8]), "+f"(d[9]), "+f"(d[10]), "+f"(d[11]), "+f"(d[12]), "+f"(d[13]), "+f"(d[14]), "+f"(d[15]), "+f"(d[16]), "+f"(d[17]), "+f"(d[18]), "+f"(d[19]), "+f"(d[20]), "+f"(d[21]), "+f"(d[22]), "+f"(d[23]), "+f"(d[24]), "+f"(d[25]), "+f"(d[26]), "+f"(d[27]), "+f"(d[28]), "+f"(d[29]), "+f"(d[30]), "+f"(d[31]), "+f"(d[32]), "+f"(d[33]), "+f"(d[34]), "+f"(d[35]), "+f"(d[36]), "+f"(d[37]), "+f"(d[38]), "+f"(d[39]), "+f"(d[40]), "+f"(d[41]), "+f"(d[42]), "+f"(d[43]), "+f"(d[44]), "+f"(d[45]), "+f"(d[46]), "+f"(d[47]), "+f"(d[48]), "+f"(d[49]), "+f"(d[50]), "+f"(d[51]), "+f"(d[52]), "+f"(d[53]), "+f"(d[54]), "+f"(d[55]), "+f"(d[56]), "+f"(d[57]), "+f"(d[58]), "+f"(d[59]), "+f"(d[60]), "+f"(d[61]), "+f"(d[62]), "+f"(d[63])
                     : "l"(a), "l"(b), "r"(acc));
    else
        asm volatile("{\n.reg .pred p;\nsetp.ne.b32 p, %66, 0;\n"
                     "wgmma.mma_async.sync.aligned.m64n128k16.f32.f16.f16 {%0,%1,%2,%3,%4,%5,%6,%7,%8,%9,%10,%11,%12,%13,%14,%15,%16,%17,%18,%19,%20,%21,%22,%23,%24,%25,%26,%27,%28,%29,%30,%31,%32,%33,%34,%35,%36,%37,%38,%39,%40,%41,%42,%43,%44,%45,%46,%47,%48,%49,%50,%51,%52,%53,%54,%55,%56,%57,%58,%59,%60,%61,%62,%63}, %64, %65, p, 1, 1, 0, 0;\n}"
                     : "+f"(d[0]), "+f"(d[1]), "+f"(d[2]), "+f"(d[3]), "+f"(d[4]), "+f"(d[5]), "+f"(d[6]), "+f"(d[7]), "+f"(d[8]), "+f"(d[9]), "+f"(d[10]), "+f"(d[11]), "+f"(d[12]), "+f"(d[13]), "+f"(d[14]), "+f"(d[15]), "+f"(d[16]), "+f"(d[17]), "+f"(d[18]), "+f"(d[19]), "+f"(d[20]), "+f"(d[21]), "+f"(d[22]), "+f"(d[23]), "+f"(d[24]), "+f"(d[25]), "+f"(d[26]), "+f"(d[27]), "+f"(d[28]), "+f"(d[29]), "+f"(d[30]), "+f"(d[31]), "+f"(d[32]), "+f"(d[33]), "+f"(d[34]), "+f"(d[35]), "+f"(d[36]), "+f"(d[37]), "+f"(d[38]), "+f"(d[39]), "+f"(d[40]), "+f"(d[41]), "+f"(d[42]), "+f"(d[43]), "+f"(d[44]), "+f"(d[45]), "+f"(d[46]), "+f"(d[47]), "+f"(d[48]), "+f"(d[49]), "+f"(d[50]), "+f"(d[51]), "+f"(d[52]), "+f"(d[53]), "+f"(d[54]), "+f"(d[55]), "+f"(d[56]), "+f"(d[57]), "+f"(d[58]), "+f"(d[59]), "+f"(d[60]), "+f"(d[61]), "+f"(d[62]), "+f"(d[63])
                     : "l"(a), "l"(b), "r"(acc));
}

template <>
__device__ __forceinline__ void wgmma_m64k16<128, true>(float* d, uint64_t a, uint64_t b, uint32_t acc, int tnsp) {
    if (tnsp)
        asm volatile("{\n.reg .pred p;\nsetp.ne.b32 p, %66, 0;\n"
                     "wgmma.mma_async.sync.aligned.m64n128k16.f32.bf16.bf16 {%0,%1,%2,%3,%4,%5,%6,%7,%8,%9,%10,%11,%12,%13,%14,%15,%16,%17,%18,%19,%20,%21,%22,%23,%24,%25,%26,%27,%28,%29,%30,%31,%32,%33,%34,%35,%36,%37,%38,%39,%40,%41,%42,%43,%44,%45,%46,%47,%48,%49,%50,%51,%52,%53,%54,%55,%56,%57,%58,%59,%60,%61,%62,%63}, %64, %65, p, 1, 1, 1, 1;\n}"
                     : "+f"(d[0]), "+f"(d[1]), "+f"(d[2]), "+f"(d[3]), "+f"(d[4]), "+f"(d[5]), "+f"(d[6]), "+f"(d[7]), "+f"(d[8]), "+f"(d[9]), "+f"(d[10]), "+f"(d[11]), "+f"(d[12]), "+f"(d[13]), "+f"(d[14]), "+f"(d[15]), "+f"(d[16]), "+f"(d[17]), "+f"(d[18]), "+f"(d[19]), "+f"(d[20]), "+f"(d[21]), "+f"(d[22]), "+f"(d[23]), "+f"(d[24]), "+f"(d[25]), "+f"(d[26]), "+f"(d[27]), "+f"(d[28]), "+f"(d[29]), "+f"(d[30]), "+f"(d[31]), "+f"(d[32]), "+f"(d[33]), "+f"(d[34]), "+f"(d[35]), "+f"(d[36]), "+f"(d[37]), "+f"(d[38]), "+f"(d[39]), "+f"(d[40]), "+f"(d[41]), "+f"(d[42]), "+f"(d[43]), "+f"(d[44]), "+f"(d[45]), "+f"(d[46]), "+f"(d[47]), "+f"(d[48]), "+f"(d[49]), "+f"(d[50]), "+f"(d[51]), "+f"(d[52]), "+f"(d[53]), "+f"(d[54]), "+f"(d[55]), "+f"(d[56]), "+f"(d[57]), "+f"(d[58]), "+f"(d[59]), "+f"(d[60]), "+f"(d[61]), "+f"(d[62]), "+f"(d[63])
                     : "l"(a), "l"(b), "r"(acc));
    else
        asm volatile("{\n.reg .pred p;\nsetp.ne.b32 p, %66, 0;\n"
                     "wgmma.mma_async.sync.aligned.m64n128k16.f32.bf16.bf16 {%0,%1,%2,%3,%4,%5,%6,%7,%8,%9,%10,%11,%12,%13,%14,%15,%16,%17,%18,%19,%20,%21,%22,%23,%24,%25,%26,%27,%28,%29,%30,%31,%32,%33,%34,%35,%36,%37,%38,%39,%40,%41,%42,%43,%44,%45,%46,%47,%48,%49,%50,%51,%52,%53,%54,%55,%56,%57,%58,%59,%60,%61,%62,%63}, %64, %65, p, 1, 1, 0, 0;\n}"
                     : "+f"(d[0]), "+f"(d[1]), "+f"(d[2]), "+f"(d[3]), "+f"(d[4]), "+f"(d[5]), "+f"(d[6]), "+f"(d[7]), "+f"(d[8]), "+f"(d[9]), "+f"(d[10]), "+f"(d[11]), "+f"(d[12]), "+f"(d[13]), "+f"(d[14]), "+f"(d[15]), "+f"(d[16]), "+f"(d[17]), "+f"(d[18]), "+f"(d[19]), "+f"(d[20]), "+f"(d[21]), "+f"(d[22]), "+f"(d[23]), "+f"(d[24]), "+f"(d[25]), "+f"(d[26]), "+f"(d[27]), "+f"(d[28]), "+f"(d[29]), "+f"(d[30]), "+f"(d[31]), "+f"(d[32]), "+f"(d[33]), "+f"(d[34]), "+f"(d[35]), "+f"(d[36]), "+f"(d[37]), "+f"(d[38]), "+f"(d[39]), "+f"(d[40]), "+f"(d[41]), "+f"(d[42]), "+f"(d[43]), "+f"(d[44]), "+f"(d[45]), "+f"(d[46]), "+f"(d[47]), "+f"(d[48]), "+f"(d[49]), "+f"(d[50]), "+f"(d[51]), "+f"(d[52]), "+f"(d[53]), "+f"(d[54]), "+f"(d[55]), "+f"(d[56]), "+f"(d[57]), "+f"(d[58]), "+f"(d[59]), "+f"(d[60]), "+f"(d[61]), "+f"(d[62]), "+f"(d[63])
                     : "l"(a), "l"(b), "r"(acc));
}

template <>
__device__ __forceinline__ void wgmma_m64k16<256, false>(float* d, uint64_t a, uint64_t b, uint32_t acc, int tnsp) {
    if (tnsp)
        asm volatile("{\n.reg .pred p;\nsetp.ne.b32 p, %130, 0;\n"
                     "wgmma.mma_async.sync.aligned.m64n256k16.f32.f16.f16 {%0,%1,%2,%3,%4,%5,%6,%7,%8,%9,%10,%11,%12,%13,%14,%15,%16,%17,%18,%19,%20,%21,%22,%23,%24,%25,%26,%27,%28,%29,%30,%31,%32,%33,%34,%35,%36,%37,%38,%39,%40,%41,%42,%43,%44,%45,%46,%47,%48,%49,%50,%51,%52,%53,%54,%55,%56,%57,%58,%59,%60,%61,%62,%63,%64,%65,%66,%67,%68,%69,%70,%71,%72,%73,%74,%75,%76,%77,%78,%79,%80,%81,%82,%83,%84,%85,%86,%87,%88,%89,%90,%91,%92,%93,%94,%95,%96,%97,%98,%99,%100,%101,%102,%103,%104,%105,%106,%107,%108,%109,%110,%111,%112,%113,%114,%115,%116,%117,%118,%119,%120,%121,%122,%123,%124,%125,%126,%127}, %128, %129, p, 1, 1, 1, 1;\n}"
                     : "+f"(d[0]), "+f"(d[1]), "+f"(d[2]), "+f"(d[3]), "+f"(d[4]), "+f"(d[5]), "+f"(d[6]), "+f"(d[7]), "+f"(d[8]), "+f"(d[9]), "+f"(d[10]), "+f"(d[11]), "+f"(d[12]), "+f"(d[13]), "+f"(d[14]), "+f"(d[15]), "+f"(d[16]), "+f"(d[17]), "+f"(d[18]), "+f"(d[19]), "+f"(d[20]), "+f"(d[21]), "+f"(d[22]), "+f"(d[23]), "+f"(d[24]), "+f"(d[25]), "+f"(d[26]), "+f"(d[27]), "+f"(d[28]), "+f"(d[29]), "+f"(d[30]), "+f"(d[31]), "+f"(d[32]), "+f"(d[33]), "+f"(d[34]), "+f"(d[35]), "+f"(d[36]), "+f"(d[37]), "+f"(d[38]), "+f"(d[39]), "+f"(d[40]), "+f"(d[41]), "+f"(d[42]), "+f"(d[43]), "+f"(d[44]), "+f"(d[45]), "+f"(d[46]), "+f"(d[47]), "+f"(d[48]), "+f"(d[49]), "+f"(d[50]), "+f"(d[51]), "+f"(d[52]), "+f"(d[53]), "+f"(d[54]), "+f"(d[55]), "+f"(d[56]), "+f"(d[57]), "+f"(d[58]), "+f"(d[59]), "+f"(d[60]), "+f"(d[61]), "+f"(d[62]), "+f"(d[63]), "+f"(d[64]), "+f"(d[65]), "+f"(d[66]), "+f"(d[67]), "+f"(d[68]), "+f"(d[69]), "+f"(d[70]), "+f"(d[71]), "+f"(d[72]), "+f"(d[73]), "+f"(d[74]), "+f"(d[75]), "+f"(d[76]), "+f"(d[77]), "+f"(d[78]), "+f"(d[79]), "+f"(d[80]), "+f"(d[81]), "+f"(d[82]), "+f"(d[83]), "+f"(d[84]), "+f"(d[85]), "+f"(d[86]), "+f"(d[87]), "+f"(d[88]), "+f"(d[89]), "+f"(d[90]), "+f"(d[91]), "+f"(d[92]), "+f"(d[93]), "+f"(d[94]), "+f"(d[95]), "+f"(d[96]), "+f"(d[97]), "+f"(d[98]), "+f"(d[99]), "+f"(d[100]), "+f"(d[101]), "+f"(d[102]), "+f"(d[103]), "+f"(d[104]), "+f"(d[105]), "+f"(d[106]), "+f"(d[107]), "+f"(d[108]), "+f"(d[109]), "+f"(d[110]), "+f"(d[111]), "+f"(d[112]), "+f"(d[113]), "+f"(d[114]), "+f"(d[115]), "+f"(d[116]), "+f"(d[117]), "+f"(d[118]), "+f"(d[119]), "+f"(d[120]), "+f"(d[121]), "+f"(d[122]), "+f"(d[123]), "+f"(d[124]), "+f"(d[125]), "+f"(d[126]), "+f"(d[127])
                     : "l"(a), "l"(b), "r"(acc));
    else
        asm volatile("{\n.reg .pred p;\nsetp.ne.b32 p, %130, 0;\n"
                     "wgmma.mma_async.sync.aligned.m64n256k16.f32.f16.f16 {%0,%1,%2,%3,%4,%5,%6,%7,%8,%9,%10,%11,%12,%13,%14,%15,%16,%17,%18,%19,%20,%21,%22,%23,%24,%25,%26,%27,%28,%29,%30,%31,%32,%33,%34,%35,%36,%37,%38,%39,%40,%41,%42,%43,%44,%45,%46,%47,%48,%49,%50,%51,%52,%53,%54,%55,%56,%57,%58,%59,%60,%61,%62,%63,%64,%65,%66,%67,%68,%69,%70,%71,%72,%73,%74,%75,%76,%77,%78,%79,%80,%81,%82,%83,%84,%85,%86,%87,%88,%89,%90,%91,%92,%93,%94,%95,%96,%97,%98,%99,%100,%101,%102,%103,%104,%105,%106,%107,%108,%109,%110,%111,%112,%113,%114,%115,%116,%117,%118,%119,%120,%121,%122,%123,%124,%125,%126,%127}, %128, %129, p, 1, 1, 0, 0;\n}"
                     : "+f"(d[0]), "+f"(d[1]), "+f"(d[2]), "+f"(d[3]), "+f"(d[4]), "+f"(d[5]), "+f"(d[6]), "+f"(d[7]), "+f"(d[8]), "+f"(d[9]), "+f"(d[10]), "+f"(d[11]), "+f"(d[12]), "+f"(d[13]), "+f"(d[14]), "+f"(d[15]), "+f"(d[16]), "+f"(d[17]), "+f"(d[18]), "+f"(d[19]), "+f"(d[20]), "+f"(d[21]), "+f"(d[22]), "+f"(d[23]), "+f"(d[24]), "+f"(d[25]), "+f"(d[26]), "+f"(d[27]), "+f"(d[28]), "+f"(d[29]), "+f"(d[30]), "+f"(d[31]), "+f"(d[32]), "+f"(d[33]), "+f"(d[34]), "+f"(d[35]), "+f"(d[36]), "+f"(d[37]), "+f"(d[38]), "+f"(d[39]), "+f"(d[40]), "+f"(d[41]), "+f"(d[42]), "+f"(d[43]), "+f"(d[44]), "+f"(d[45]), "+f"(d[46]), "+f"(d[47]), "+f"(d[48]), "+f"(d[49]), "+f"(d[50]), "+f"(d[51]), "+f"(d[52]), "+f"(d[53]), "+f"(d[54]), "+f"(d[55]), "+f"(d[56]), "+f"(d[57]), "+f"(d[58]), "+f"(d[59]), "+f"(d[60]), "+f"(d[61]), "+f"(d[62]), "+f"(d[63]), "+f"(d[64]), "+f"(d[65]), "+f"(d[66]), "+f"(d[67]), "+f"(d[68]), "+f"(d[69]), "+f"(d[70]), "+f"(d[71]), "+f"(d[72]), "+f"(d[73]), "+f"(d[74]), "+f"(d[75]), "+f"(d[76]), "+f"(d[77]), "+f"(d[78]), "+f"(d[79]), "+f"(d[80]), "+f"(d[81]), "+f"(d[82]), "+f"(d[83]), "+f"(d[84]), "+f"(d[85]), "+f"(d[86]), "+f"(d[87]), "+f"(d[88]), "+f"(d[89]), "+f"(d[90]), "+f"(d[91]), "+f"(d[92]), "+f"(d[93]), "+f"(d[94]), "+f"(d[95]), "+f"(d[96]), "+f"(d[97]), "+f"(d[98]), "+f"(d[99]), "+f"(d[100]), "+f"(d[101]), "+f"(d[102]), "+f"(d[103]), "+f"(d[104]), "+f"(d[105]), "+f"(d[106]), "+f"(d[107]), "+f"(d[108]), "+f"(d[109]), "+f"(d[110]), "+f"(d[111]), "+f"(d[112]), "+f"(d[113]), "+f"(d[114]), "+f"(d[115]), "+f"(d[116]), "+f"(d[117]), "+f"(d[118]), "+f"(d[119]), "+f"(d[120]), "+f"(d[121]), "+f"(d[122]), "+f"(d[123]), "+f"(d[124]), "+f"(d[125]), "+f"(d[126]), "+f"(d[127])
                     : "l"(a), "l"(b), "r"(acc));
}

template <>
__device__ __forceinline__ void wgmma_m64k16<256, true>(float* d, uint64_t a, uint64_t b, uint32_t acc, int tnsp) {
    if (tnsp)
        asm volatile("{\n.reg .pred p;\nsetp.ne.b32 p, %130, 0;\n"
                     "wgmma.mma_async.sync.aligned.m64n256k16.f32.bf16.bf16 {%0,%1,%2,%3,%4,%5,%6,%7,%8,%9,%10,%11,%12,%13,%14,%15,%16,%17,%18,%19,%20,%21,%22,%23,%24,%25,%26,%27,%28,%29,%30,%31,%32,%33,%34,%35,%36,%37,%38,%39,%40,%41,%42,%43,%44,%45,%46,%47,%48,%49,%50,%51,%52,%53,%54,%55,%56,%57,%58,%59,%60,%61,%62,%63,%64,%65,%66,%67,%68,%69,%70,%71,%72,%73,%74,%75,%76,%77,%78,%79,%80,%81,%82,%83,%84,%85,%86,%87,%88,%89,%90,%91,%92,%93,%94,%95,%96,%97,%98,%99,%100,%101,%102,%103,%104,%105,%106,%107,%108,%109,%110,%111,%112,%113,%114,%115,%116,%117,%118,%119,%120,%121,%122,%123,%124,%125,%126,%127}, %128, %129, p, 1, 1, 1, 1;\n}"
                     : "+f"(d[0]), "+f"(d[1]), "+f"(d[2]), "+f"(d[3]), "+f"(d[4]), "+f"(d[5]), "+f"(d[6]), "+f"(d[7]), "+f"(d[8]), "+f"(d[9]), "+f"(d[10]), "+f"(d[11]), "+f"(d[12]), "+f"(d[13]), "+f"(d[14]), "+f"(d[15]), "+f"(d[16]), "+f"(d[17]), "+f"(d[18]), "+f"(d[19]), "+f"(d[20]), "+f"(d[21]), "+f"(d[22]), "+f"(d[23]), "+f"(d[24]), "+f"(d[25]), "+f"(d[26]), "+f"(d[27]), "+f"(d[28]), "+f"(d[29]), "+f"(d[30]), "+f"(d[31]), "+f"(d[32]), "+f"(d[33]), "+f"(d[34]), "+f"(d[35]), "+f"(d[36]), "+f"(d[37]), "+f"(d[38]), "+f"(d[39]), "+f"(d[40]), "+f"(d[41]), "+f"(d[42]), "+f"(d[43]), "+f"(d[44]), "+f"(d[45]), "+f"(d[46]), "+f"(d[47]), "+f"(d[48]), "+f"(d[49]), "+f"(d[50]), "+f"(d[51]), "+f"(d[52]), "+f"(d[53]), "+f"(d[54]), "+f"(d[55]), "+f"(d[56]), "+f"(d[57]), "+f"(d[58]), "+f"(d[59]), "+f"(d[60]), "+f"(d[61]), "+f"(d[62]), "+f"(d[63]), "+f"(d[64]), "+f"(d[65]), "+f"(d[66]), "+f"(d[67]), "+f"(d[68]), "+f"(d[69]), "+f"(d[70]), "+f"(d[71]), "+f"(d[72]), "+f"(d[73]), "+f"(d[74]), "+f"(d[75]), "+f"(d[76]), "+f"(d[77]), "+f"(d[78]), "+f"(d[79]), "+f"(d[80]), "+f"(d[81]), "+f"(d[82]), "+f"(d[83]), "+f"(d[84]), "+f"(d[85]), "+f"(d[86]), "+f"(d[87]), "+f"(d[88]), "+f"(d[89]), "+f"(d[90]), "+f"(d[91]), "+f"(d[92]), "+f"(d[93]), "+f"(d[94]), "+f"(d[95]), "+f"(d[96]), "+f"(d[97]), "+f"(d[98]), "+f"(d[99]), "+f"(d[100]), "+f"(d[101]), "+f"(d[102]), "+f"(d[103]), "+f"(d[104]), "+f"(d[105]), "+f"(d[106]), "+f"(d[107]), "+f"(d[108]), "+f"(d[109]), "+f"(d[110]), "+f"(d[111]), "+f"(d[112]), "+f"(d[113]), "+f"(d[114]), "+f"(d[115]), "+f"(d[116]), "+f"(d[117]), "+f"(d[118]), "+f"(d[119]), "+f"(d[120]), "+f"(d[121]), "+f"(d[122]), "+f"(d[123]), "+f"(d[124]), "+f"(d[125]), "+f"(d[126]), "+f"(d[127])
                     : "l"(a), "l"(b), "r"(acc));
    else
        asm volatile("{\n.reg .pred p;\nsetp.ne.b32 p, %130, 0;\n"
                     "wgmma.mma_async.sync.aligned.m64n256k16.f32.bf16.bf16 {%0,%1,%2,%3,%4,%5,%6,%7,%8,%9,%10,%11,%12,%13,%14,%15,%16,%17,%18,%19,%20,%21,%22,%23,%24,%25,%26,%27,%28,%29,%30,%31,%32,%33,%34,%35,%36,%37,%38,%39,%40,%41,%42,%43,%44,%45,%46,%47,%48,%49,%50,%51,%52,%53,%54,%55,%56,%57,%58,%59,%60,%61,%62,%63,%64,%65,%66,%67,%68,%69,%70,%71,%72,%73,%74,%75,%76,%77,%78,%79,%80,%81,%82,%83,%84,%85,%86,%87,%88,%89,%90,%91,%92,%93,%94,%95,%96,%97,%98,%99,%100,%101,%102,%103,%104,%105,%106,%107,%108,%109,%110,%111,%112,%113,%114,%115,%116,%117,%118,%119,%120,%121,%122,%123,%124,%125,%126,%127}, %128, %129, p, 1, 1, 0, 0;\n}"
                     : "+f"(d[0]), "+f"(d[1]), "+f"(d[2]), "+f"(d[3]), "+f"(d[4]), "+f"(d[5]), "+f"(d[6]), "+f"(d[7]), "+f"(d[8]), "+f"(d[9]), "+f"(d[10]), "+f"(d[11]), "+f"(d[12]), "+f"(d[13]), "+f"(d[14]), "+f"(d[15]), "+f"(d[16]), "+f"(d[17]), "+f"(d[18]), "+f"(d[19]), "+f"(d[20]), "+f"(d[21]), "+f"(d[22]), "+f"(d[23]), "+f"(d[24]), "+f"(d[25]), "+f"(d[26]), "+f"(d[27]), "+f"(d[28]), "+f"(d[29]), "+f"(d[30]), "+f"(d[31]), "+f"(d[32]), "+f"(d[33]), "+f"(d[34]), "+f"(d[35]), "+f"(d[36]), "+f"(d[37]), "+f"(d[38]), "+f"(d[39]), "+f"(d[40]), "+f"(d[41]), "+f"(d[42]), "+f"(d[43]), "+f"(d[44]), "+f"(d[45]), "+f"(d[46]), "+f"(d[47]), "+f"(d[48]), "+f"(d[49]), "+f"(d[50]), "+f"(d[51]), "+f"(d[52]), "+f"(d[53]), "+f"(d[54]), "+f"(d[55]), "+f"(d[56]), "+f"(d[57]), "+f"(d[58]), "+f"(d[59]), "+f"(d[60]), "+f"(d[61]), "+f"(d[62]), "+f"(d[63]), "+f"(d[64]), "+f"(d[65]), "+f"(d[66]), "+f"(d[67]), "+f"(d[68]), "+f"(d[69]), "+f"(d[70]), "+f"(d[71]), "+f"(d[72]), "+f"(d[73]), "+f"(d[74]), "+f"(d[75]), "+f"(d[76]), "+f"(d[77]), "+f"(d[78]), "+f"(d[79]), "+f"(d[80]), "+f"(d[81]), "+f"(d[82]), "+f"(d[83]), "+f"(d[84]), "+f"(d[85]), "+f"(d[86]), "+f"(d[87]), "+f"(d[88]), "+f"(d[89]), "+f"(d[90]), "+f"(d[91]), "+f"(d[92]), "+f"(d[93]), "+f"(d[94]), "+f"(d[95]), "+f"(d[96]), "+f"(d[97]), "+f"(d[98]), "+f"(d[99]), "+f"(d[100]), "+f"(d[101]), "+f"(d[102]), "+f"(d[103]), "+f"(d[104]), "+f"(d[105]), "+f"(d[106]), "+f"(d[107]), "+f"(d[108]), "+f"(d[109]), "+f"(d[110]), "+f"(d[111]), "+f"(d[112]), "+f"(d[113]), "+f"(d[114]), "+f"(d[115]), "+f"(d[116]), "+f"(d[117]), "+f"(d[118]), "+f"(d[119]), "+f"(d[120]), "+f"(d[121]), "+f"(d[122]), "+f"(d[123]), "+f"(d[124]), "+f"(d[125]), "+f"(d[126]), "+f"(d[127])
                     : "l"(a), "l"(b), "r"(acc));
}
template <int CW>
__device__ __forceinline__ void acc_to_rows(const float* acc0, const float* acc1, int c0, float* xb, uint32_t bar_id, uint32_t* v) {
    constexpr int P = CW + 1;
    const int t = threadIdx.x & 127, w = t >> 5, l = t & 31;
#pragma unroll
    for (int h = 0; h < 2; ++h) {
        const float* a = h ? acc1 : acc0;
        const int r0 = 64 * h + 16 * w + (l >> 2);
#pragma unroll
        for (int j = 0; j < CW / 8; ++j) {
            const int col = 8 * j + 2 * (l & 3);
            const int i = (c0 / 8 + j) * 4;
            xb[r0 * P + col] = a[i];
            xb[r0 * P + col + 1] = a[i + 1];
            xb[(r0 + 8) * P + col] = a[i + 2];
            xb[(r0 + 8) * P + col + 1] = a[i + 3];
        }
    }
    asm volatile("bar.sync %0, 128;" ::"r"(bar_id) : "memory");
#pragma unroll
    for (int c = 0; c < CW; ++c) v[c] = __float_as_uint(xb[t * P + c]);
    asm volatile("bar.sync %0, 128;" ::"r"(bar_id) : "memory");
}
template <int CW>
__host__ __device__ constexpr int xbuf_bytes() { return (128 * (CW + 1) * 4 + 1023) / 1024 * 1024; }

}
```

Baseline: 61210.

## Add patch-fed channel-major conv path loading one haloed input patch per tile

Adds a patch-fed variant of the channel-major implicit-GEMM conv. It loads one haloed 10x26 input patch per tile and channel chunk into a small ring of slots, then addresses each tap as an offset view into that patch. This replaces per-tap A-tile loads, so input bytes are read once rather than once per tap. The tile becomes 8x24 = 192 pixels, which needs new m64n192 wgmma specializations and a templated epilogue size. The residual prefetch also moves from after the epilogue to a point early in the next tile's mainloop. The patch slots take shared memory away from the pipeline stages, and the smaller tile means more tiles per layer.

New measurement: 62720, median of 6. +2.5%, better.

```diff
diff --git a/wav2lip_b200/csrc/conv_igemm.cuh b/wav2lip_b200/csrc/conv_igemm.cuh
--- a/wav2lip_b200/csrc/conv_igemm.cuh
+++ b/wav2lip_b200/csrc/conv_igemm.cuh
@@ -48,6 +48,8 @@
     int sx, sy;
     int ntaps, kc_per_tap;
     unsigned stage_tx_bytes;
+    int pox, poy;
+    unsigned patch_tx_bytes;
     EpiParams ep;
     int a_lo_off;
     signed char dx[kMaxSteps];
@@ -119,11 +121,16 @@
 }
 
 constexpr int kCmPixels = 256;
-template <int BN, int BK, int MT = 1, bool kCM = false>
+constexpr int kCpTileW = 8, kCpTileH = 24, kCpPixels = kCpTileW * kCpTileH;
+constexpr int kCpPW = kCpTileW + 2, kCpPH = kCpTileH + 2;
+constexpr int kCpChunks = 2, kCpSlots = 3;
+constexpr int kCpSlot = (kCpPW * kCpPH * 64 * 2 + 1023) / 1024 * 1024;
+template <int BN, int BK, int MT = 1, bool kCM = false, bool kPF = false>
 struct ConvCfg {
-    static constexpr int kRowsA = kCM ? kCmPixels : kTileM;
+    static constexpr int kRowsA = kPF ? kCpPixels : kCM ? kCmPixels : kTileM;
     static constexpr int kATile = kRowsA * BK * 2;
-    static constexpr int kABytes = MT * kATile;
+    static constexpr int kABytes = kPF ? 0 : MT * kATile;
+    static constexpr int kPatchBytes = kPF ? kCpSlots * kCpSlot : 0;
     static constexpr int kBBytes = BN * BK * 2;
     static constexpr int kStageBytes = kABytes + kBBytes;
     static constexpr int kEW = BN < 64 ? BN : 64;
@@ -132,13 +139,14 @@
     static constexpr int kBoxBytes = kRowsA * kEW * 2;
     static constexpr int kGrpRaw = (kCM || kPasses * kBoxBytes > xbuf_bytes<kCW>()) ? kPasses * kBoxBytes : xbuf_bytes<kCW>();
     static constexpr int kGrpBytes = (kGrpRaw + 1023) / 1024 * 1024;
-    static constexpr int kStagesRaw = (kSmemMax - kSmemExtra - 2 * kGrpBytes) / kStageBytes;
+    static constexpr int kStagesRaw = (kSmemMax - kSmemExtra - 2 * kGrpBytes - kPatchBytes) / kStageBytes;
     static constexpr int kStages = kStagesRaw > 8 ? 8 : kStagesRaw;
     static constexpr int kRingBytes = (kStages * kStageBytes + 1023) / 1024 * 1024;
-    static constexpr int kSmemBytes = kRingBytes + 2 * kGrpBytes + kSmemExtra;
+    static constexpr int kSmemBytes = kRingBytes + kPatchBytes + 2 * kGrpBytes + kSmemExtra;
     static constexpr int kThreads = 384;
     static_assert(BN <= 128, "a warpgroup holds at most 128 fp32 accumulator columns per row");
     static_assert(!kCM || (BN == 128 && BK == 64 && MT == 1), "channel-major form: 128 channels, 128-byte K rows, one tile");
+    static_assert(!kPF || kCM, "the patch-fed form is a channel-major form");
     static_assert(kBoxBytes % 1024 == 0, "staging boxes must keep the 1024-byte swizzle alignment");
     static_assert(kStages >= 2, "need a pipeline");
     static_assert(kSmemBytes <= kSmemMax, "shared-memory carve-up exceeds the per-CTA limit");
@@ -269,8 +277,8 @@
 __device__ __forceinline__ void named_bar_sync(uint32_t id, uint32_t n) { asm volatile("bar.sync %0, %1;" ::"r"(id), "r"(n) : "memory"); }
 __device__ __forceinline__ void named_bar_arrive(uint32_t id, uint32_t n) { asm volatile("bar.arrive %0, %1;" ::"r"(id), "r"(n) : "memory"); }
 
-template <bool kBF16, typename AfterRes, typename Live>
-__device__ __forceinline__ void chmajor_epilogue(float (&acc)[128], float sc0, float sh0, float sc1, float sh1, int act,
+template <bool kBF16, int NACC, typename AfterRes, typename Live>
+__device__ __forceinline__ void chmajor_epilogue(float (&acc)[NACC], float sc0, float sh0, float sc1, float sh1, int act,
                                                  uint32_t res, int res_pitch, AfterRes&& after_res, Live&& live, uint32_t stg,
                                                  uint32_t bar_id, bool leader, const CUtensorMap* tmO, int c0, int c1, int c2,
                                                  int c3) {
@@ -279,7 +287,7 @@
     const int lm_row = lane >> 4, lm_px = lane & 7;
     const uint32_t lm_chunk = 16u * (2 * q + ((lane >> 3) & 1));
 #pragma unroll
-    for (int i = 0; i < 16; ++i) {
+    for (int i = 0; i < NACC / 8; ++i) {
 #pragma unroll
         for (int h = 0; h < 2; ++h) {
             float* a = acc + 8 * i + 4 * h;
@@ -303,15 +311,15 @@
     after_res();
     if (act == ACT_RELU) {
 #pragma unroll
-        for (int j = 0; j < 128; ++j) acc[j] = fmaxf(acc[j], 0.0f);
+        for (int j = 0; j < NACC; ++j) acc[j] = fmaxf(acc[j], 0.0f);
     } else if (act == ACT_LRELU) {
 #pragma unroll
-        for (int j = 0; j < 128; ++j) acc[j] = acc[j] > 0.0f ? acc[j] : 0.01f * acc[j];
+        for (int j = 0; j < NACC; ++j) acc[j] = acc[j] > 0.0f ? acc[j] : 0.01f * acc[j];
     }
     if (leader) asm volatile("cp.async.bulk.wait_group.read 0;" ::: "memory");
     named_bar_sync(bar_id, 128);
 #pragma unroll
-    for (int i = 0; i < 16; ++i) {
+    for (int i = 0; i < NACC / 8; ++i) {
         uint32_t ad = stg + static_cast<uint32_t>((2 * i + lm_row) * 8 + lm_px) * kRowB + lm_chunk;
         ad ^= ((ad >> 7) & 7u) << 4;
         const uint32_t l0 = live(2 * i), l1 = live(2 * i + 1);
@@ -338,10 +346,10 @@
 template <int kRegs>
 __device__ __forceinline__ void setmaxnreg_inc() { asm volatile("setmaxnreg.inc.sync.aligned.u32 %0;" ::"n"(kRegs)); }
 
-template <int BN, int BK, bool kBF16, bool kHead, int MT = 1, bool kCM = false>
-__global__ void __launch_bounds__(ConvCfg<BN, BK, MT, kCM>::kThreads, 1) conv_igemm_kernel(const __grid_constant__ ConvParams p) {
+template <int BN, int BK, bool kBF16, bool kHead, int MT = 1, bool kCM = false, bool kPF = false>
+__global__ void __launch_bounds__(ConvCfg<BN, BK, MT, kCM, kPF>::kThreads, 1) conv_igemm_kernel(const __grid_constant__ ConvParams p) {
     pdl_launch_dependents();
-    using Cfg = ConvCfg<BN, BK, MT, kCM>;
+    using Cfg = ConvCfg<BN, BK, MT, kCM, kPF>;
     constexpr int kStages = Cfg::kStages;
     static_assert(!kHead || BN == 32, "fused head expects the 32-channel output block");
     static_assert(MT == 1 || MT == 2, "one or two M tiles per unit");
@@ -350,11 +358,14 @@
     extern __shared__ uint8_t smem_raw[];
     const uint32_t smem_raw_u32 = smem_u32(smem_raw);
     const uint32_t smem_base = (smem_raw_u32 + 1023u) & ~1023u;
-    const uint32_t grp_base = smem_base + Cfg::kRingBytes;
+    const uint32_t patch_base = smem_base + Cfg::kRingBytes;
+    const uint32_t grp_base = patch_base + Cfg::kPatchBytes;
     const uint32_t bar_base = grp_base + 2 * Cfg::kGrpBytes;
     auto full_bar = [&](int s) { return bar_base + 8u * s; };
     auto empty_bar = [&](int s) { return bar_base + 8u * (kStages + s); };
     auto res_bar = [&](int g) { return bar_base + 8u * (2 * kStages + g); };
+    auto pfull_bar = [&](int s) { return bar_base + 8u * (2 * kStages + 2 + s); };
+    auto pempty_bar = [&](int s) { return bar_base + 8u * (2 * kStages + 2 + kCpSlots + s); };
 
     const int warp = threadIdx.x >> 5;
     const int lane = threadIdx.x & 31;
@@ -373,6 +384,12 @@
             mbar_init(empty_bar(s), kCM ? 8 : 4 * MT);
         }
         for (int g = 0; g < 2; ++g) mbar_init(res_bar(g), 1);
+        if constexpr (kPF) {
+            for (int s = 0; s < kCpSlots; ++s) {
+                mbar_init(pfull_bar(s), 1);
+                mbar_init(pempty_bar(s), 8);
+            }
+        }
         fence_barrier_init();
     }
     __syncthreads();
@@ -385,7 +402,34 @@
 
     if (warp < 4) {
         setmaxnreg_dec<kProducerRegs>();
-        if (warp == 0 && lane == 0) {
+        if constexpr (kPF) {
+            if (warp == 0 && lane == 0) {
+                int stage = 0;
+                uint32_t phase = 0;
+                int pj = 0;
+                for (int tile = blockIdx.x; tile < total_tiles; tile += gridDim.x) {
+                    const int nt = tile % p.n_tiles;
+                    const int m = tile / p.n_tiles;
+                    const int x0 = (m % p.tiles_x) * kCpTileW + p.pox;
+                    const int y0 = ((m / p.tiles_x) % p.tiles_y) * kCpTileH + p.poy;
+                    const int n0 = m / (p.tiles_x * p.tiles_y);
+                    for (int kc = 0; kc < kCpChunks; ++kc, ++pj) {
+                        const int slot = pj % kCpSlots;
+                        mbar_wait(pempty_bar(slot), (static_cast<uint32_t>(pj / kCpSlots) & 1u) ^ 1u);
+                        mbar_arrive_expect_tx(pfull_bar(slot), p.patch_tx_bytes);
+                        tma_load_4d(patch_base + slot * kCpSlot, &p.tmA, pfull_bar(slot), kc * BK, x0, y0, n0);
+                    }
+                    for (int t = 0; t < p.ntaps; ++t) {
+                        for (int kc = 0; kc < kCpChunks; ++kc) {
+                            mbar_wait(empty_bar(stage), phase ^ 1u);
+                            mbar_arrive_expect_tx(full_bar(stage), p.stage_tx_bytes);
+                            tma_load_3d(smem_base + stage * Cfg::kStageBytes, &p.tmB, full_bar(stage), kc * BK, nt * BN, p.b_slab[t]);
+                            if (++stage == kStages) { stage = 0; phase ^= 1u; }
+                        }
+                    }
+                }
+            }
+        } else if (warp == 0 && lane == 0) {
             int stage = 0;
             uint32_t phase = 0;
             for (int tile = blockIdx.x; tile < total_tiles; tile += gridDim.x) {
@@ -428,6 +472,7 @@
         const bool has_res = p.ep.res != nullptr;
         const int rows_valid = p.bw * p.bh * p.bn;
         const int ch = 64 * g + 16 * q + (lane >> 2);
+        constexpr int kPx = Cfg::kRowsA;
         auto tile_origin = [&](int tile_, int* nt_, int* x0_, int* y0_, int* n0_) {
             *nt_ = tile_ % p.n_tiles;
             const int m_ = tile_ / p.n_tiles;
@@ -435,46 +480,76 @@
             *y0_ = ((m_ / p.tiles_x) % p.tiles_y) * p.bh;
             *n0_ = (m_ / (p.tiles_x * p.tiles_y)) * p.bn;
         };
+        constexpr int kResStep = 2;
         auto fetch_res = [&](int tile_) {
+            asm volatile("cp.async.bulk.wait_group.read 0;" ::: "memory");
             int nt_, x0_, y0_, n0_;
             tile_origin(tile_, &nt_, &x0_, &y0_, &n0_);
             mbar_arrive_expect_tx(res_bar(g), p.epi_box_bytes);
             tma_load_4d(stg, &p.tmR, res_bar(g), nt_ * BN + 64 * g, x0_, y0_, n0_);
         };
-        if (has_res && leader && static_cast<int>(blockIdx.x) < total_tiles) fetch_res(blockIdx.x);
-        float acc[128];
+        float acc[kPx / 2];
         int stage = 0;
         uint32_t phase = 0, rphase = 0;
-        for (int tile = blockIdx.x; tile < total_tiles; tile += gridDim.x) {
+        for (int tile = blockIdx.x, it = 0; tile < total_tiles; tile += gridDim.x, ++it) {
             int prev = -1;
-            for (int ks = 0; ks < k_steps; ++ks) {
-                mbar_wait(full_bar(stage), phase);
-                const uint32_t box = smem_base + stage * Cfg::kStageBytes;
-                const uint32_t wts = box + Cfg::kABytes + g * (64 * BK * 2);
-                wg_fence();
-#pragma unroll
-                for (int k = 0; k < BK / 16; ++k)
-                    wgmma_m64k16<256, kBF16>(acc, make_kmajor_desc<BK>(wts + 32u * k), make_kmajor_desc<BK>(box + 32u * k),
-                                             (ks | k) != 0 ? 1u : 0u, 0);
-                wg_commit();
-                wg_wait<1>();
-                if (prev >= 0 && lane == 0) mbar_arrive(empty_bar(prev));
-                prev = stage;
-                if (++stage == kStages) { stage = 0; phase ^= 1u; }
+            if constexpr (kPF) {
+                const int pj0 = kCpChunks * it;
+                for (int t = 0; t < p.ntaps; ++t) {
+                    const uint32_t tap_off = static_cast<uint32_t>((p.dy[t] - p.poy) * kCpPW + (p.dx[t] - p.pox)) * (BK * 2);
+#pragma unroll
+                    for (int kc = 0; kc < kCpChunks; ++kc) {
+                        const int slot = (pj0 + kc) % kCpSlots;
+                        if (t == 0) mbar_wait(pfull_bar(slot), static_cast<uint32_t>((pj0 + kc) / kCpSlots) & 1u);
+                        mbar_wait(full_bar(stage), phase);
+                        const uint32_t wts = smem_base + stage * Cfg::kStageBytes + g * (64 * BK * 2);
+                        const uint32_t view = patch_base + slot * kCpSlot + tap_off;
+                        wg_fence();
+#pragma unroll
+                        for (int k = 0; k < BK / 16; ++k)
+                            wgmma_m64k16<kPx, kBF16>(acc, make_kmajor_desc<BK>(wts + 32u * k),
+                                                     wg_desc(view + 32u * k, 16, kCpPW * BK * 2, BK * 2), (t | kc | k) != 0 ? 1u : 0u, 0);
+                        wg_commit();
+                        if (has_res && leader && kCpChunks * t + kc == kResStep) fetch_res(tile);
+                        wg_wait<1>();
+                        if (prev >= 0 && lane == 0) mbar_arrive(empty_bar(prev));
+                        if (kc == 1 && t == p.ntaps - 1 && lane == 0) mbar_arrive(pempty_bar(pj0 % kCpSlots));
+                        prev = stage;
+                        if (++stage == kStages) { stage = 0; phase ^= 1u; }
+                    }
+                }
+            } else {
+                for (int ks = 0; ks < k_steps; ++ks) {
+                    mbar_wait(full_bar(stage), phase);
+                    const uint32_t box = smem_base + stage * Cfg::kStageBytes;
+                    const uint32_t wts = box + Cfg::kABytes + g * (64 * BK * 2);
+                    wg_fence();
+#pragma unroll
+                    for (int k = 0; k < BK / 16; ++k)
+                        wgmma_m64k16<kPx, kBF16>(acc, make_kmajor_desc<BK>(wts + 32u * k), make_kmajor_desc<BK>(box + 32u * k),
+                                                 (ks | k) != 0 ? 1u : 0u, 0);
+                    wg_commit();
+                    if (has_res && leader && ks == kResStep) fetch_res(tile);
+                    wg_wait<1>();
+                    if (prev >= 0 && lane == 0) mbar_arrive(empty_bar(prev));
+                    prev = stage;
+                    if (++stage == kStages) { stage = 0; phase ^= 1u; }
+                }
             }
             wg_wait<0>();
-            wg_fence_regs<128>(acc);
+            wg_fence_regs<kPx / 2>(acc);
             if (lane == 0) mbar_arrive(empty_bar(prev));
+            if (kPF && lane == 0) mbar_arrive(pempty_bar((kCpChunks * it + 1) % kCpSlots));
 
             int nt, x0, y0, n0;
             tile_origin(tile, &nt, &x0, &y0, &n0);
             uint64_t live = ~0ull;
             if constexpr (!kBF16) {
                 const int xr = p.ep.Wout - x0, yr = p.ep.Hout - y0, nr = p.ep.N - n0;
-                if (rows_valid < kCmPixels || xr < p.bw || yr < p.bh || nr < p.bn) {
+                if (rows_valid < kPx || xr < p.bw || yr < p.bh || nr < p.bn) {
                     live = 0;
 #pragma unroll 1
-                    for (int b = 0; b < 64; ++b) {
+                    for (int b = 0; b < kPx / 4; ++b) {
                         const int px = 8 * (b >> 1) + 2 * (lane & 3) + (b & 1);
                         const int xx = px % p.bw, yy = (px / p.bw) % p.bh, nn = px / (p.bw * p.bh);
                         if (px < rows_valid && xx < xr && yy < yr && nn < nr) live |= 1ull << b;
@@ -493,10 +568,6 @@
                     return (static_cast<uint32_t>(live >> (2 * j)) & 1u) << 15 | (static_cast<uint32_t>(live >> (2 * j + 1)) & 1u) << 31;
                 },
                 stg, bar_id, leader, &p.tmO, nt * BN + 64 * g, x0, y0, n0);
-            if (has_res && leader && tile + static_cast<int>(gridDim.x) < total_tiles) {
-                asm volatile("cp.async.bulk.wait_group.read 0;" ::: "memory");
-                fetch_res(tile + gridDim.x);
-            }
         }
         if (leader) asm volatile("cp.async.bulk.wait_group 0;" ::: "memory");
     } else {
diff --git a/wav2lip_b200/csrc/host_launch.cuh b/wav2lip_b200/csrc/host_launch.cuh
--- a/wav2lip_b200/csrc/host_launch.cuh
+++ b/wav2lip_b200/csrc/host_launch.cuh
@@ -1,7 +1,7 @@
 #pragma once
 
 typedef void (*ConvKernelFn)(const ConvParams);
-struct ConvKernelEntry { int BN, BK; bool bf16, head; ConvKernelFn fn; int smem; uint64_t attr_set; int mt; int threads; bool cm; };
+struct ConvKernelEntry { int BN, BK; bool bf16, head; ConvKernelFn fn; int smem; uint64_t attr_set; int mt; int threads; bool cm; bool pf; };
 
 #define W2L_CONV_ENTRY(BN_, BK_)                                                                                                        \
     {BN_, BK_, false, false, conv_igemm_kernel<BN_, BK_, false, false>, ConvCfg<BN_, BK_>::kSmemBytes, 0, 1, ConvCfg<BN_, BK_>::kThreads, false}, \
@@ -12,6 +12,9 @@
 #define W2L_CONV_ENTRY_CM(BN_, BK_)                                                                                                     \
     {BN_, BK_, false, false, conv_igemm_kernel<BN_, BK_, false, false, 1, true>, ConvCfg<BN_, BK_, 1, true>::kSmemBytes, 0, 1, ConvCfg<BN_, BK_, 1, true>::kThreads, true}, \
     {BN_, BK_, true, false, conv_igemm_kernel<BN_, BK_, true, false, 1, true>, ConvCfg<BN_, BK_, 1, true>::kSmemBytes, 0, 1, ConvCfg<BN_, BK_, 1, true>::kThreads, true}
+#define W2L_CONV_ENTRY_PF(BN_, BK_)                                                                                                     \
+    {BN_, BK_, false, false, conv_igemm_kernel<BN_, BK_, false, false, 1, true, true>, ConvCfg<BN_, BK_, 1, true, true>::kSmemBytes, 0, 1, ConvCfg<BN_, BK_, 1, true, true>::kThreads, true, true}, \
+    {BN_, BK_, true, false, conv_igemm_kernel<BN_, BK_, true, false, 1, true, true>, ConvCfg<BN_, BK_, 1, true, true>::kSmemBytes, 0, 1, ConvCfg<BN_, BK_, 1, true, true>::kThreads, true, true}
 
 static ConvKernelEntry g_conv_kernels[] = {
     W2L_CONV_ENTRY(16, 16), W2L_CONV_ENTRY(16, 32), W2L_CONV_ENTRY(16, 64),
@@ -19,14 +22,14 @@
     W2L_CONV_ENTRY(64, 16), W2L_CONV_ENTRY(64, 32), W2L_CONV_ENTRY(64, 64),
     W2L_CONV_ENTRY(128, 16), W2L_CONV_ENTRY(128, 32), W2L_CONV_ENTRY(128, 64),
     W2L_CONV_ENTRY_MT2(64, 64), W2L_CONV_ENTRY_MT2(64, 32),
-    W2L_CONV_ENTRY_CM(128, 64),
+    W2L_CONV_ENTRY_CM(128, 64), W2L_CONV_ENTRY_PF(128, 64),
     {32, 16, false, true, conv_igemm_kernel<32, 16, false, true>, ConvCfg<32, 16>::kSmemBytes, 0, 1, ConvCfg<32, 16>::kThreads, false},
     {32, 16, true, true, conv_igemm_kernel<32, 16, true, true>, ConvCfg<32, 16>::kSmemBytes, 0, 1, ConvCfg<32, 16>::kThreads, false},
 };
 
-static ConvKernelEntry* find_conv_kernel(int BN, int BK, bool bf16, bool head, int mt = 1, bool cm = false) {
+static ConvKernelEntry* find_conv_kernel(int BN, int BK, bool bf16, bool head, int mt = 1, bool cm = false, bool pf = false) {
     for (auto& e : g_conv_kernels)
-        if (e.BN == BN && e.BK == BK && e.bf16 == bf16 && e.head == head && e.mt == mt && e.cm == cm) return &e;
+        if (e.BN == BN && e.BK == BK && e.bf16 == bf16 && e.head == head && e.mt == mt && e.cm == cm && e.pf == pf) return &e;
     return nullptr;
 }
 
@@ -109,8 +112,8 @@
         ctx->launches++;
         return W2L_OK;
     }
-    ConvKernelEntry* e = find_conv_kernel(op.BN, op.BK, ctx->bf16, op.head, op.MT, op.cm);
-    if (!e) return fail(W2L_EINVAL, "no conv kernel for BN=%d BK=%d head=%d MT=%d cm=%d", op.BN, op.BK, (int)op.head, op.MT, (int)op.cm);
+    ConvKernelEntry* e = find_conv_kernel(op.BN, op.BK, ctx->bf16, op.head, op.MT, op.cm, op.pf);
+    if (!e) return fail(W2L_EINVAL, "no conv kernel for BN=%d BK=%d head=%d MT=%d cm=%d pf=%d", op.BN, op.BK, (int)op.head, op.MT, (int)op.cm, (int)op.pf);
     CKR(ensure_smem_attr(&e->attr_set, ctx->device, (const void*)e->fn, e->smem));
     CK(launch_k(e->fn, op.grid, e->threads, (size_t)e->smem, st, op.cp, pdl));
     ctx->launches++;
diff --git a/wav2lip_b200/csrc/host_ops.cuh b/wav2lip_b200/csrc/host_ops.cuh
--- a/wav2lip_b200/csrc/host_ops.cuh
+++ b/wav2lip_b200/csrc/host_ops.cuh
@@ -223,6 +223,7 @@
     else
         while (BN > 32 && m_tiles * (a.cout / BN) < ctx->num_sms && a.cout % (BN / 2) == 0) BN /= 2;
     const int k_steps = w.ntaps * (w.cin_pad / BK);
+    int pox = 0, poy = 0;
     if (ctx->use_tma_epi && !ctx->x2 && !a.head && !a.out.f32 && a.cout % 128 == 0 && w.cout_pad % 128 == 0 && BK == 64 &&
         a.osx == 1 && a.osy == 1 && k_steps >= kCmMinSteps) {
         int cw, ch, cn;
@@ -236,11 +237,24 @@
         if ((cm_tiles * nt + S - 1) / S * k_steps >= kCmMinCtaSteps &&
             fill(cm_tiles, kCmPixels) >= (1.0 - kCmFillMargin) * fill(m_tiles, kTileM)) {
             op.cm = true;
-            op.name += " [cm]";
             BN = 128;
             bw = cw; bh = ch; bn = cn;
+            int mnx = 127, mxx = -127, mny = 127, mxy = -127;
+            for (int t = 0; t < w.ntaps; ++t) {
+                mnx = std::min(mnx, (int)w.dx[t]); mxx = std::max(mxx, (int)w.dx[t]);
+                mny = std::min(mny, (int)w.dy[t]); mxy = std::max(mxy, (int)w.dy[t]);
+            }
+            const long long pf_tiles = (long long)((a.Wl + kCpTileW - 1) / kCpTileW) * ((a.Hl + kCpTileH - 1) / kCpTileH) * a.in.N;
+            if (ctx->use_patch && a.sx == 1 && a.sy == 1 && w.cin_pad == kCpChunks * BK && mxx - mnx <= kCpPW - kCpTileW &&
+                mxy - mny <= kCpPH - kCpTileH && fill(pf_tiles, kCpPixels) >= (1.0 - kCmFillMargin) * fill(cm_tiles, kCmPixels)) {
+                op.pf = true;
+                op.name += " [patch-fed]";
+                bw = kCpTileW; bh = kCpTileH; bn = 1;
+            }
+            op.name += " [cm]";
             tiles_x = (a.Wl + bw - 1) / bw; tiles_y = (a.Hl + bh - 1) / bh; tiles_n = (a.in.N + bn - 1) / bn;
             m_tiles = tiles_x * tiles_y * tiles_n;
+            pox = mnx; poy = mny;
         }
     }
     if (w.cout_pad % BN != 0) return fail(W2L_EINVAL, "%s: cout_pad %d vs BN %d", a.name.c_str(), w.cout_pad, BN);
@@ -253,13 +267,18 @@
 
     ConvParams& p = op.cp;
     memset(&p, 0, sizeof(p));
-    CKR(encode_act_map(ctx, &p.tmA, a.in, BK, bw * a.sx, bh * a.sy, bn, a.sx, a.sy, a.name.c_str()));
+    if (op.pf)
+        CKR(encode_act_map(ctx, &p.tmA, a.in, BK, kCpPW, kCpPH, 1, 1, 1, a.name.c_str()));
+    else
+        CKR(encode_act_map(ctx, &p.tmA, a.in, BK, bw * a.sx, bh * a.sy, bn, a.sx, a.sy, a.name.c_str()));
     CKR(encode_w_map(ctx, &p.tmB, w, BK, BN, a.name.c_str()));
     p.tiles_x = tiles_x; p.tiles_y = tiles_y; p.tiles_n = tiles_n; p.n_tiles = a.cout / BN;
     p.bw = bw; p.bh = bh; p.bn = bn;
     p.sx = a.sx; p.sy = a.sy;
     p.ntaps = w.ntaps; p.kc_per_tap = w.cin_pad / BK;
-    p.stage_tx_bytes = (unsigned)(op.MT * bw * bh * bn * BK * 2 + BN * BK * 2);
+    p.stage_tx_bytes = (unsigned)((op.pf ? 0 : op.MT * bw * bh * bn * BK * 2) + BN * BK * 2);
+    p.pox = pox; p.poy = poy;
+    p.patch_tx_bytes = op.pf ? (unsigned)(kCpPW * kCpPH * BK * 2) : 0u;
     fill_epi(&p.ep, a);
     p.tma_epi = 0;
     if (ctx->use_tma_epi && !ctx->x2 && !a.head && !a.out.f32) {
diff --git a/wav2lip_b200/csrc/host_types.h b/wav2lip_b200/csrc/host_types.h
--- a/wav2lip_b200/csrc/host_types.h
+++ b/wav2lip_b200/csrc/host_types.h
@@ -155,6 +155,7 @@
     ConvParams cp;
     int BN = 0, BK = 0, MT = 1;
     bool cm = false;
+    bool pf = false;
     bool head = false;
     int grid = 0;
     double flops = 0;
diff --git a/wav2lip_b200/csrc/wgmma.cuh b/wav2lip_b200/csrc/wgmma.cuh
--- a/wav2lip_b200/csrc/wgmma.cuh
+++ b/wav2lip_b200/csrc/wgmma.cuh
@@ -135,6 +135,34 @@
         asm volatile("{\n.reg .pred p;\nsetp.ne.b32 p, %66, 0;\n"
                      "wgmma.mma_async.sync.aligned.m64n128k16.f32.bf16.bf16 {%0,%1,%2,%3,%4,%5,%6,%7,%8,%9,%10,%11,%12,%13,%14,%15,%16,%17,%18,%19,%20,%21,%22,%23,%24,%25,%26,%27,%28,%29,%30,%31,%32,%33,%34,%35,%36,%37,%38,%39,%40,%41,%42,%43,%44,%45,%46,%47,%48,%49,%50,%51,%52,%53,%54,%55,%56,%57,%58,%59,%60,%61,%62,%63}, %64, %65, p, 1, 1, 0, 0;\n}"
                      : "+f"(d[0]), "+f"(d[1]), "+f"(d[2]), "+f"(d[3]), "+f"(d[4]), "+f"(d[5]), "+f"(d[6]), "+f"(d[7]), "+f"(d[8]), "+f"(d[9]), "+f"(d[10]), "+f"(d[11]), "+f"(d[12]), "+f"(d[13]), "+f"(d[14]), "+f"(d[15]), "+f"(d[16]), "+f"(d[17]), "+f"(d[18]), "+f"(d[19]), "+f"(d[20]), "+f"(d[21]), "+f"(d[22]), "+f"(d[23]), "+f"(d[24]), "+f"(d[25]), "+f"(d[26]), "+f"(d[27]), "+f"(d[28]), "+f"(d[29]), "+f"(d[30]), "+f"(d[31]), "+f"(d[32]), "+f"(d[33]), "+f"(d[34]), "+f"(d[35]), "+f"(d[36]), "+f"(d[37]), "+f"(d[38]), "+f"(d[39]), "+f"(d[40]), "+f"(d[41]), "+f"(d[42]), "+f"(d[43]), "+f"(d[44]), "+f"(d[45]), "+f"(d[46]), "+f"(d[47]), "+f"(d[48]), "+f"(d[49]), "+f"(d[50]), "+f"(d[51]), "+f"(d[52]), "+f"(d[53]), "+f"(d[54]), "+f"(d[55]), "+f"(d[56]), "+f"(d[57]), "+f"(d[58]), "+f"(d[59]), "+f"(d[60]), "+f"(d[61]), "+f"(d[62]), "+f"(d[63])
+                     : "l"(a), "l"(b), "r"(acc));
+}
+
+template <>
+__device__ __forceinline__ void wgmma_m64k16<192, false>(float* d, uint64_t a, uint64_t b, uint32_t acc, int tnsp) {
+    if (tnsp)
+        asm volatile("{\n.reg .pred p;\nsetp.ne.b32 p, %98, 0;\n"
+                     "wgmma.mma_async.sync.aligned.m64n192k16.f32.f16.f16 {%0,%1,%2,%3,%4,%5,%6,%7,%8,%9,%10,%11,%12,%13,%14,%15,%16,%17,%18,%19,%20,%21,%22,%23,%24,%25,%26,%27,%28,%29,%30,%31,%32,%33,%34,%35,%36,%37,%38,%39,%40,%41,%42,%43,%44,%45,%46,%47,%48,%49,%50,%51,%52,%53,%54,%55,%56,%57,%58,%59,%60,%61,%62,%63,%64,%65,%66,%67,%68,%69,%70,%71,%72,%73,%74,%75,%76,%77,%78,%79,%80,%81,%82,%83,%84,%85,%86,%87,%88,%89,%90,%91,%92,%93,%94,%95}, %96, %97, p, 1, 1, 1, 1;\n}"
+                     : "+f"(d[0]), "+f"(d[1]), "+f"(d[2]), "+f"(d[3]), "+f"(d[4]), "+f"(d[5]), "+f"(d[6]), "+f"(d[7]), "+f"(d[8]), "+f"(d[9]), "+f"(d[10]), "+f"(d[11]), "+f"(d[12]), "+f"(d[13]), "+f"(d[14]), "+f"(d[15]), "+f"(d[16]), "+f"(d[17]), "+f"(d[18]), "+f"(d[19]), "+f"(d[20]), "+f"(d[21]), "+f"(d[22]), "+f"(d[23]), "+f"(d[24]), "+f"(d[25]), "+f"(d[26]), "+f"(d[27]), "+f"(d[28]), "+f"(d[29]), "+f"(d[30]), "+f"(d[31]), "+f"(d[32]), "+f"(d[33]), "+f"(d[34]), "+f"(d[35]), "+f"(d[36]), "+f"(d[37]), "+f"(d[38]), "+f"(d[39]), "+f"(d[40]), "+f"(d[41]), "+f"(d[42]), "+f"(d[43]), "+f"(d[44]), "+f"(d[45]), "+f"(d[46]), "+f"(d[47]), "+f"(d[48]), "+f"(d[49]), "+f"(d[50]), "+f"(d[51]), "+f"(d[52]), "+f"(d[53]), "+f"(d[54]), "+f"(d[55]), "+f"(d[56]), "+f"(d[57]), "+f"(d[58]), "+f"(d[59]), "+f"(d[60]), "+f"(d[61]), "+f"(d[62]), "+f"(d[63]), "+f"(d[64]), "+f"(d[65]), "+f"(d[66]), "+f"(d[67]), "+f"(d[68]), "+f"(d[69]), "+f"(d[70]), "+f"(d[71]), "+f"(d[72]), "+f"(d[73]), "+f"(d[74]), "+f"(d[75]), "+f"(d[76]), "+f"(d[77]), "+f"(d[78]), "+f"(d[79]), "+f"(d[80]), "+f"(d[81]), "+f"(d[82]), "+f"(d[83]), "+f"(d[84]), "+f"(d[85]), "+f"(d[86]), "+f"(d[87]), "+f"(d[88]), "+f"(d[89]), "+f"(d[90]), "+f"(d[91]), "+f"(d[92]), "+f"(d[93]), "+f"(d[94]), "+f"(d[95])
+                     : "l"(a), "l"(b), "r"(acc));
+    else
+        asm volatile("{\n.reg .pred p;\nsetp.ne.b32 p, %98, 0;\n"
+                     "wgmma.mma_async.sync.aligned.m64n192k16.f32.f16.f16 {%0,%1,%2,%3,%4,%5,%6,%7,%8,%9,%10,%11,%12,%13,%14,%15,%16,%17,%18,%19,%20,%21,%22,%23,%24,%25,%26,%27,%28,%29,%30,%31,%32,%33,%34,%35,%36,%37,%38,%39,%40,%41,%42,%43,%44,%45,%46,%47,%48,%49,%50,%51,%52,%53,%54,%55,%56,%57,%58,%59,%60,%61,%62,%63,%64,%65,%66,%67,%68,%69,%70,%71,%72,%73,%74,%75,%76,%77,%78,%79,%80,%81,%82,%83,%84,%85,%86,%87,%88,%89,%90,%91,%92,%93,%94,%95}, %96, %97, p, 1, 1, 0, 0;\n}"
+                     : "+f"(d[0]), "+f"(d[1]), "+f"(d[2]), "+f"(d[3]), "+f"(d[4]), "+f"(d[5]), "+f"(d[6]), "+f"(d[7]), "+f"(d[8]), "+f"(d[9]), "+f"(d[10]), "+f"(d[11]), "+f"(d[12]), "+f"(d[13]), "+f"(d[14]), "+f"(d[15]), "+f"(d[16]), "+f"(d[17]), "+f"(d[18]), "+f"(d[19]), "+f"(d[20]), "+f"(d[21]), "+f"(d[22]), "+f"(d[23]), "+f"(d[24]), "+f"(d[25]), "+f"(d[26]), "+f"(d[27]), "+f"(d[28]), "+f"(d[29]), "+f"(d[30]), "+f"(d[31]), "+f"(d[32]), "+f"(d[33]), "+f"(d[34]), "+f"(d[35]), "+f"(d[36]), "+f"(d[37]), "+f"(d[38]), "+f"(d[39]), "+f"(d[40]), "+f"(d[41]), "+f"(d[42]), "+f"(d[43]), "+f"(d[44]), "+f"(d[45]), "+f"(d[46]), "+f"(d[47]), "+f"(d[48]), "+f"(d[49]), "+f"(d[50]), "+f"(d[51]), "+f"(d[52]), "+f"(d[53]), "+f"(d[54]), "+f"(d[55]), "+f"(d[56]), "+f"(d[57]), "+f"(d[58]), "+f"(d[59]), "+f"(d[60]), "+f"(d[61]), "+f"(d[62]), "+f"(d[63]), "+f"(d[64]), "+f"(d[65]), "+f"(d[66]), "+f"(d[67]), "+f"(d[68]), "+f"(d[69]), "+f"(d[70]), "+f"(d[71]), "+f"(d[72]), "+f"(d[73]), "+f"(d[74]), "+f"(d[75]), "+f"(d[76]), "+f"(d[77]), "+f"(d[78]), "+f"(d[79]), "+f"(d[80]), "+f"(d[81]), "+f"(d[82]), "+f"(d[83]), "+f"(d[84]), "+f"(d[85]), "+f"(d[86]), "+f"(d[87]), "+f"(d[88]), "+f"(d[89]), "+f"(d[90]), "+f"(d[91]), "+f"(d[92]), "+f"(d[93]), "+f"(d[94]), "+f"(d[95])
+                     : "l"(a), "l"(b), "r"(acc));
+}
+
+template <>
+__device__ __forceinline__ void wgmma_m64k16<192, true>(float* d, uint64_t a, uint64_t b, uint32_t acc, int tnsp) {
+    if (tnsp)
+        asm volatile("{\n.reg .pred p;\nsetp.ne.b32 p, %98, 0;\n"
+                     "wgmma.mma_async.sync.aligned.m64n192k16.f32.bf16.bf16 {%0,%1,%2,%3,%4,%5,%6,%7,%8,%9,%10,%11,%12,%13,%14,%15,%16,%17,%18,%19,%20,%21,%22,%23,%24,%25,%26,%27,%28,%29,%30,%31,%32,%33,%34,%35,%36,%37,%38,%39,%40,%41,%42,%43,%44,%45,%46,%47,%48,%49,%50,%51,%52,%53,%54,%55,%56,%57,%58,%59,%60,%61,%62,%63,%64,%65,%66,%67,%68,%69,%70,%71,%72,%73,%74,%75,%76,%77,%78,%79,%80,%81,%82,%83,%84,%85,%86,%87,%88,%89,%90,%91,%92,%93,%94,%95}, %96, %97, p, 1, 1, 1, 1;\n}"
+                     : "+f"(d[0]), "+f"(d[1]), "+f"(d[2]), "+f"(d[3]), "+f"(d[4]), "+f"(d[5]), "+f"(d[6]), "+f"(d[7]), "+f"(d[8]), "+f"(d[9]), "+f"(d[10]), "+f"(d[11]), "+f"(d[12]), "+f"(d[13]), "+f"(d[14]), "+f"(d[15]), "+f"(d[16]), "+f"(d[17]), "+f"(d[18]), "+f"(d[19]), "+f"(d[20]), "+f"(d[21]), "+f"(d[22]), "+f"(d[23]), "+f"(d[24]), "+f"(d[25]), "+f"(d[26]), "+f"(d[27]), "+f"(d[28]), "+f"(d[29]), "+f"(d[30]), "+f"(d[31]), "+f"(d[32]), "+f"(d[33]), "+f"(d[34]), "+f"(d[35]), "+f"(d[36]), "+f"(d[37]), "+f"(d[38]), "+f"(d[39]), "+f"(d[40]), "+f"(d[41]), "+f"(d[42]), "+f"(d[43]), "+f"(d[44]), "+f"(d[45]), "+f"(d[46]), "+f"(d[47]), "+f"(d[48]), "+f"(d[49]), "+f"(d[50]), "+f"(d[51]), "+f"(d[52]), "+f"(d[53]), "+f"(d[54]), "+f"(d[55]), "+f"(d[56]), "+f"(d[57]), "+f"(d[58]), "+f"(d[59]), "+f"(d[60]), "+f"(d[61]), "+f"(d[62]), "+f"(d[63]), "+f"(d[64]), "+f"(d[65]), "+f"(d[66]), "+f"(d[67]), "+f"(d[68]), "+f"(d[69]), "+f"(d[70]), "+f"(d[71]), "+f"(d[72]), "+f"(d[73]), "+f"(d[74]), "+f"(d[75]), "+f"(d[76]), "+f"(d[77]), "+f"(d[78]), "+f"(d[79]), "+f"(d[80]), "+f"(d[81]), "+f"(d[82]), "+f"(d[83]), "+f"(d[84]), "+f"(d[85]), "+f"(d[86]), "+f"(d[87]), "+f"(d[88]), "+f"(d[89]), "+f"(d[90]), "+f"(d[91]), "+f"(d[92]), "+f"(d[93]), "+f"(d[94]), "+f"(d[95])
+                     : "l"(a), "l"(b), "r"(acc));
+    else
+        asm volatile("{\n.reg .pred p;\nsetp.ne.b32 p, %98, 0;\n"
+                     "wgmma.mma_async.sync.aligned.m64n192k16.f32.bf16.bf16 {%0,%1,%2,%3,%4,%5,%6,%7,%8,%9,%10,%11,%12,%13,%14,%15,%16,%17,%18,%19,%20,%21,%22,%23,%24,%25,%26,%27,%28,%29,%30,%31,%32,%33,%34,%35,%36,%37,%38,%39,%40,%41,%42,%43,%44,%45,%46,%47,%48,%49,%50,%51,%52,%53,%54,%55,%56,%57,%58,%59,%60,%61,%62,%63,%64,%65,%66,%67,%68,%69,%70,%71,%72,%73,%74,%75,%76,%77,%78,%79,%80,%81,%82,%83,%84,%85,%86,%87,%88,%89,%90,%91,%92,%93,%94,%95}, %96, %97, p, 1, 1, 0, 0;\n}"
+                     : "+f"(d[0]), "+f"(d[1]), "+f"(d[2]), "+f"(d[3]), "+f"(d[4]), "+f"(d[5]), "+f"(d[6]), "+f"(d[7]), "+f"(d[8]), "+f"(d[9]), "+f"(d[10]), "+f"(d[11]), "+f"(d[12]), "+f"(d[13]), "+f"(d[14]), "+f"(d[15]), "+f"(d[16]), "+f"(d[17]), "+f"(d[18]), "+f"(d[19]), "+f"(d[20]), "+f"(d[21]), "+f"(d[22]), "+f"(d[23]), "+f"(d[24]), "+f"(d[25]), "+f"(d[26]), "+f"(d[27]), "+f"(d[28]), "+f"(d[29]), "+f"(d[30]), "+f"(d[31]), "+f"(d[32]), "+f"(d[33]), "+f"(d[34]), "+f"(d[35]), "+f"(d[36]), "+f"(d[37]), "+f"(d[38]), "+f"(d[39]), "+f"(d[40]), "+f"(d[41]), "+f"(d[42]), "+f"(d[43]), "+f"(d[44]), "+f"(d[45]), "+f"(d[46]), "+f"(d[47]), "+f"(d[48]), "+f"(d[49]), "+f"(d[50]), "+f"(d[51]), "+f"(d[52]), "+f"(d[53]), "+f"(d[54]), "+f"(d[55]), "+f"(d[56]), "+f"(d[57]), "+f"(d[58]), "+f"(d[59]), "+f"(d[60]), "+f"(d[61]), "+f"(d[62]), "+f"(d[63]), "+f"(d[64]), "+f"(d[65]), "+f"(d[66]), "+f"(d[67]), "+f"(d[68]), "+f"(d[69]), "+f"(d[70]), "+f"(d[71]), "+f"(d[72]), "+f"(d[73]), "+f"(d[74]), "+f"(d[75]), "+f"(d[76]), "+f"(d[77]), "+f"(d[78]), "+f"(d[79]), "+f"(d[80]), "+f"(d[81]), "+f"(d[82]), "+f"(d[83]), "+f"(d[84]), "+f"(d[85]), "+f"(d[86]), "+f"(d[87]), "+f"(d[88]), "+f"(d[89]), "+f"(d[90]), "+f"(d[91]), "+f"(d[92]), "+f"(d[93]), "+f"(d[94]), "+f"(d[95])
                      : "l"(a), "l"(b), "r"(acc));
 }
 
```
